# powdr-labs/powdr

Measured on AMD Instinct MI355X. Metric: STARK cells/sec (trace rows x cols) proving guest-keccak [bus interactions (LogUp) inside the proof], higher is better.
Workload: dtype u32 (BabyBear, Montgomery)

## Files before the change

include/powdr_prover.h:

```cpp
#ifndef POWDR_PROVER_H
#define POWDR_PROVER_H

#include <stddef.h>
#include <stdint.h>

#ifdef __cplusplus
extern "C" {
#endif

typedef struct PwProver PwProver;

typedef struct {
    uint32_t num_queries;
    uint32_t pow_bits;
} PwStarkConfig;

PwProver* pw_prover_create(const PwStarkConfig* cfg, uint32_t width, const uint32_t* cons_bytecode,
                           size_t bytecode_len, const uint32_t* cons_spans, size_t n_constraints);
PwProver* pw_prover_create_logup(const PwStarkConfig* cfg, uint32_t width, const uint32_t* cons_bytecode,
                                 size_t bytecode_len, const uint32_t* cons_spans, size_t n_constraints,
                                 const uint32_t* interactions, size_t n_interactions, const uint32_t* inter_spans,
                                 size_t n_inter_spans, const uint32_t* inter_bytecode, size_t inter_bytecode_len);
int pw_prover_trace_root(PwProver* p, const uint32_t* d_trace, uint32_t log_height, uint32_t* root8);
int pw_prover_set_bus_seed(PwProver* p, const uint32_t* seed8);
// ... 112 lines not shown

void pw_set_device_budget(size_t bytes);
size_t pw_get_device_budget(void);

int pw_prove_airs(const PwSegmentAir* airs, size_t n_airs, int shared_bus_seed, unsigned n_workers,
                  const uint32_t** proofs, size_t* n_words, uint32_t* bus_seed8);

typedef struct PwAirDescription {
    uint32_t width, log_height;
    uint32_t logup;
    const uint32_t* cons_bytecode; size_t bytecode_len;
    const uint32_t* cons_spans; size_t n_constraints;
    const uint32_t* interactions; size_t n_interactions;
    const uint32_t* inter_spans; size_t n_inter_spans;
    const uint32_t* inter_bytecode; size_t inter_bytecode_len;
} PwAirDescription;

int pw_verify_segment(const PwStarkConfig* cfg, const PwAirDescription* airs, size_t n_airs, int logup,
                      const uint32_t* proof_words, size_t n_words, int check_balance, uint32_t* total_sum4);

typedef struct PwAirPreprocessed {
    uint32_t width;
    uint32_t root8[8];
} PwAirPreprocessed;

int pw_verify_segment_preprocessed(const PwStarkConfig* cfg, const PwAirDescription* airs, const PwAirPreprocessed* pre, size_t n_airs,
                                   int logup, const uint32_t* proof_words, size_t n_words, int check_balance, uint32_t* total_sum4);

int pw_verify_segment_transition(const PwStarkConfig* cfg, const PwAirDescription* airs, const PwAirPreprocessed* pre, size_t n_airs,
                                 int logup, const uint32_t* proof_words, size_t n_words, int check_balance, uint32_t* total_sum4);

typedef struct PwAirPublic {
    uint32_t n;
    const uint32_t* expected;
} PwAirPublic;

int pw_verify_segment_public(const PwStarkConfig* cfg, const PwAirDescription* airs, const PwAirPreprocessed* pre, const PwAirPublic* pub,
                             size_t n_airs, int logup, const uint32_t* proof_words, size_t n_words, int check_balance, uint32_t* total_sum4);
size_t pw_segment_proof_public_values(const PwAirDescription* airs, const PwAirPublic* pub, size_t n_airs, const uint32_t* proof_words,
                                      size_t n_words, size_t air, uint32_t* out, size_t cap);

typedef struct PwChainSegment {
    const PwAirDescription* airs;
    const PwAirPreprocessed* pre;
    const PwAirPublic* pub;
    size_t n_airs;
    int logup;
    const uint32_t* proof;
    size_t n_words;
    int check_balance;
} PwChainSegment;
typedef struct PwChainLink {
    uint32_t air_from, index_from, air_to, index_to;
} PwChainLink;
int pw_verify_segment_chain(const PwStarkConfig* cfg, const PwChainSegment* segments, size_t n_segments, const PwChainLink* links,
                            size_t n_links, size_t* where);

int pw_verify_airs(const PwStarkConfig* cfg, const PwAirDescription* airs, size_t n_airs,
                   const uint32_t* const* proofs, const size_t* n_words, int shared_bus_seed, int check_balance,
                   uint32_t* total_sum4);

typedef int (*PwSegmentProveFn)(void* user, size_t segment, size_t worker, int device, uint32_t* commitment8);
int pw_prove_segments_multi(const int* devices, size_t n_workers, const uint64_t* segment_cells, size_t n_segments,
                            PwSegmentProveFn prove, void* user, uint32_t* commitments, uint32_t* worker_of_segment);
int pw_multi_last_merge(void);
size_t pw_assign_units(const uint64_t* cells, size_t n_units, size_t n_workers, uint32_t* worker_of_unit);

void pw_commitment_digest(const uint32_t* roots8, size_t n, uint32_t* digest8);

int pw_prover_reserve(PwProver* p, uint32_t log_height);

int pw_prover_stream_log_blocks(const PwProver* p, uint32_t log_height);

int pw_prover_max_constraint_degree(const PwProver* p);

int pw_prover_specialise(PwProver* p);
size_t pw_provers_specialise(PwProver* const* provers, size_t n);
int pw_prover_specialised(const PwProver* p, size_t* n_kernels, size_t* code_bytes, size_t* n_chunks);
size_t pw_jit_generated_source(uint32_t width, const uint32_t* cons_bytecode, size_t bytecode_len, const uint32_t* cons_spans, size_t n_constraints,
                               const uint32_t* interactions, size_t n_interactions, const uint32_t* inter_spans, size_t n_inter_spans,
                               const uint32_t* inter_bytecode, size_t inter_bytecode_len, int which, uint32_t chunk_cost, uint32_t chunks_per_unit,
                               size_t unit, char* buf, size_t cap, char* kernel_name, size_t name_cap, uint32_t* first_chunk, uint32_t* n_chunks,
                               uint32_t* total_chunks);
void pw_jit_cache_stats(uint64_t* units_compiled, uint64_t* units_from_disk);
int pw_jit_compile_check(uint32_t width, const uint32_t* cons_bytecode, size_t bytecode_len, const uint32_t* cons_spans, size_t n_constraints,
                         const uint32_t* interactions, size_t n_interactions, const uint32_t* inter_spans, size_t n_inter_spans,
                         const uint32_t* inter_bytecode, size_t inter_bytecode_len, size_t* n_kernels, size_t* code_bytes, size_t* n_chunks,
                         char* err, size_t err_cap);

uint32_t pw_prover_width(const PwProver* p);

size_t pw_prover_device_bytes(const PwProver* p);


int pw_lde_batch(const uint32_t* d_trace, uint32_t width, uint32_t log_height, uint32_t* d_coeffs, uint32_t* d_lde);

int pw_lde_fused(const uint32_t* d_trace, uint32_t width, uint32_t log_height, uint32_t* d_tmp, uint32_t* d_lde);

int pw_lde_subcoset(const uint32_t* d_coeffs, uint32_t width, uint32_t log_height, uint32_t log_blocks, uint32_t r, uint32_t* d_scale,
                    uint32_t* d_out);

int pw_merkle_commit(const uint32_t* d_matrix, size_t height, uint32_t width, uint32_t* d_digests);

void pw_poseidon2_permute_host(uint32_t* state16);

int pw_set_poseidon2_constants(const uint32_t* ext_rc, const uint32_t* int_rc);
void pw_get_poseidon2_constants(uint32_t* ext_rc, uint32_t* int_rc, uint32_t* diag);

#ifdef __cplusplus
}
#endif
#endif
```

powdr_amd/csrc/host/jit.cpp:

```cpp
#include "../jit.hpp"
#include "../common.hpp"

#include <dlfcn.h>
#include <fcntl.h>
#include <sys/file.h>
#include <spawn.h>
#include <sys/stat.h>
#include <sys/wait.h>
#include <unistd.h>

#include <atomic>
#include <cerrno>
#include <cstdio>
#include <cstdlib>
#include <cstring>
#include <iterator>
#include <map>
#include <mutex>
#include <thread>
#include <unordered_map>

extern char** environ;

namespace pw { namespace jit {
// ... 260 lines not shown
    if (!f) return;
    const uint64_t env = environment_hash(), src_len = source.size(), code_len = code.size();
    bool ok = fwrite(kDiskMagic, 1, 8, f) == 8 && fwrite(&env, 8, 1, f) == 1 && fwrite(&src_len, 8, 1, f) == 1 &&
              fwrite(source.data(), 1, source.size(), f) == source.size() && fwrite(&code_len, 8, 1, f) == 1 &&
              fwrite(code.data(), 1, code.size(), f) == code.size();
    ok = fclose(f) == 0 && ok;
    if (!ok || rename(tmp.c_str(), path.c_str()) != 0) (void)unlink(tmp.c_str());
}
}

bool compile_to_code_object(const std::string& source, std::vector<char>& code, std::string* err) { return compile_code(source, code, err); }

void cache_stats(uint64_t* compiled, uint64_t* from_disk) {
    if (compiled) *compiled = g_units_compiled.load();
    if (from_disk) *from_disk = g_units_from_disk.load();
}

bool available() {
    if (const char* e = getenv("POWDR_JIT")) if (atoi(e) == 0) return false;
    return rtc().ok;
}

std::vector<ProgramPtr> compile_all(const std::vector<std::string>& sources, std::string* err) {
    std::vector<ProgramPtr> out(sources.size());
    if (!rtc().ok) { if (err) *err = "hiprtc is not available"; return {}; }
    std::vector<size_t> todo;
    {
        std::lock_guard<std::mutex> lk(g_cache_mu);
        for (size_t i = 0; i < sources.size(); ++i) {
            auto it = g_cache.find(hash64(sources[i]));
            ProgramPtr hit = it != g_cache.end() ? it->second.lock() : nullptr;
            if (hit && hit->source == sources[i]) out[i] = hit;
            else todo.push_back(i);
        }
    }
    const std::string cache_dir = todo.empty() ? std::string() : disk_cache_dir();
    std::vector<std::pair<size_t, std::vector<char>>> from_disk;
    if (!cache_dir.empty()) {
        std::vector<size_t> still;
        for (size_t i : todo) {
            std::vector<char> c;
            if (disk_load(cache_dir, sources[i], c)) from_disk.emplace_back(i, std::move(c));
            else still.push_back(i);
        }
        todo.swap(still);
        g_units_from_disk += from_disk.size();
    }
    auto publish = [&](size_t i, std::vector<char>&& code_i) {
        auto p = std::make_shared<Program>();
        p->source = sources[i];
        p->code = std::move(code_i);
        std::weak_ptr<Program>& slot = g_cache[hash64(sources[i])];
        ProgramPtr other = slot.lock();
        if (other && other->source == sources[i]) out[i] = other;
        else { slot = p; out[i] = p; }
    };
    if (!from_disk.empty()) {
        std::lock_guard<std::mutex> lk(g_cache_mu);
        for (auto& e : from_disk) publish(e.first, std::move(e.second));
    }
    if (!todo.empty()) {
        DirLock lock(cache_dir);
        if (lock.fd >= 0) {
            std::vector<size_t> still;
            std::vector<std::pair<size_t, std::vector<char>>> late;
            for (size_t i : todo) {
                std::vector<char> c;
                if (disk_load(cache_dir, sources[i], c)) late.emplace_back(i, std::move(c));
                else still.push_back(i);
            }
            todo.swap(still);
            g_units_from_disk += late.size();
            std::lock_guard<std::mutex> lk(g_cache_mu);
            for (auto& e : late) publish(e.first, std::move(e.second));
        }
        if (!todo.empty()) {
            unsigned n_procs = std::thread::hardware_concurrency();
            if (n_procs > 32) n_procs = 32;
            if (const char* e = getenv("POWDR_JIT_THREADS")) { const int v = atoi(e); if (v >= 1 && v <= 256) n_procs = (unsigned)v; }
            if (n_procs < 1) n_procs = 1;
            if (n_procs > todo.size()) n_procs = (unsigned)todo.size();
            std::vector<std::vector<char>> code(todo.size());
            bool compiled = false;
            const std::string helper = n_procs > 1 ? helper_path() : std::string();
            std::string e;
            if (!helper.empty() && compile_with_helpers(helper, sources, todo, n_procs, code, compiled, &e)) {
                if (!compiled) { if (err) *err = e; return {}; }
            } else {
                for (size_t k = 0; k < todo.size(); ++k)
                    if (!compile_code(sources[todo[k]], code[k], &e)) { if (err) *err = e; return {}; }
            }
            g_units_compiled += todo.size();
            for (size_t k = 0; k < todo.size(); ++k) disk_store(cache_dir, sources[todo[k]], code[k]);
            std::lock_guard<std::mutex> lk(g_cache_mu);
            for (size_t k = 0; k < todo.size(); ++k) publish(todo[k], std::move(code[k]));
            if (g_cache.size() > 4096)
                for (auto it = g_cache.begin(); it != g_cache.end();) it = it->second.expired() ? g_cache.erase(it) : std::next(it);
        }
    }
    return out;
}

hipFunction_t kernel(Program& p, const char* name, std::string* err) {
    int device = 0;
    if (hipGetDevice(&device) != hipSuccess) { if (err) *err = "hipGetDevice failed"; return nullptr; }
    std::lock_guard<std::mutex> lk(p.mu);
    auto it = p.modules.find(device);
    if (it == p.modules.end()) {
        hipModule_t m = nullptr;
        const hipError_t e = hipModuleLoadData(&m, p.code.data());
        if (e != hipSuccess) { if (err) *err = std::string("hipModuleLoadData: ") + hipGetErrorString(e); (void)hipGetLastError(); return nullptr; }
        it = p.modules.emplace(device, m).first;
    }
    hipFunction_t f = nullptr;
    const hipError_t e = hipModuleGetFunction(&f, it->second, name);
    if (e != hipSuccess) { if (err) *err = std::string("hipModuleGetFunction(") + name + "): " + hipGetErrorString(e); (void)hipGetLastError(); return nullptr; }
    return f;
}

int launch(hipFunction_t f, dim3 grid, dim3 block, void** args, hipStream_t st) {
    return (int)hipModuleLaunchKernel(f, grid.x, grid.y, grid.z, block.x, block.y, block.z, 0, st, args, nullptr);
}

size_t code_bytes(const Program& p) { return p.code.size(); }

}}
```

powdr_amd/csrc/host/jit_codegen.cpp:

```cpp
#include "../jit_codegen.hpp"
#include "../xbc.hpp"

#include <cstdio>
#include <unordered_map>

namespace pw { namespace jit {

namespace {

struct Emitter {
    std::string& out;
    const char* matrix;
    std::unordered_map<uint32_t, uint32_t> loaded;
    uint32_t n_tmp = 0;
    explicit Emitter(std::string& o, const char* m) : out(o), matrix(m) {}

    std::string col(uint32_t c) {
        char b[96];
        if (!loaded.count(c)) {
            loaded[c] = 1;
            snprintf(b, sizeof b, "const uint32_t c%u = pwj::ld(%s + (size_t)%uu * N, j4);\n", c, matrix, c);
            out += b;
        }
        snprintf(b, sizeof b, "c%u", c);
        return b;
    }
    std::unordered_map<uint32_t, uint32_t> pub_loaded;
    std::string pubv(uint32_t k) {
        char b[96];
        if (!pub_loaded.count(k)) {
            pub_loaded[k] = 1;
            snprintf(b, sizeof b, "const uint32_t p%u = pub[%uu];\n", k, k);
            out += b;
        }
        snprintf(b, sizeof b, "p%u", k);
        return b;
    }
    static std::string lit(uint32_t m) { char b[24]; snprintf(b, sizeof b, "%uu", m); return b; }
    std::string tmp(const std::string& expr) {
        char b[32];
        snprintf(b, sizeof b, "t%u", n_tmp++);
        out += "const uint32_t ";
        out += b;
        out += " = " + expr + ";\n";
        return b;
    }
    bool expr(const uint32_t* code, uint32_t n_instr, std::string& value) {
        std::vector<std::string> stk;
        std::string top = "0u";
        auto bin = [&](const char* f, const std::string& a, const std::string& b) { return tmp(std::string("bb::") + f + "(" + a + ", " + b + ")"); };
        for (uint32_t ip = 0; ip < n_instr; ++ip) {
            const uint32_t op = code[2 * ip], a = code[2 * ip + 1];
            switch (op) {
                case xbc::SET_COL: top = col(a); break;
                case xbc::SET_CONST: top = lit(a); break;
                case xbc::PUSH_COL: stk.push_back(top); top = col(a); break;
                case xbc::PUSH_CONST: stk.push_back(top); top = lit(a); break;
                case xbc::ADD_COL: top = bin("add", top, col(a)); break;
                case xbc::SUB_COL: top = bin("sub", top, col(a)); break;
                case xbc::RSUB_COL: top = bin("sub", col(a), top); break;
                case xbc::MUL_COL: top = bin("mul", top, col(a)); break;
                case xbc::ADD_CONST: top = bin("add", top, lit(a)); break;
                case xbc::RSUB_CONST: top = bin("sub", lit(a), top); break;
                case xbc::MUL_CONST: top = bin("mul", top, lit(a)); break;
                case xbc::ADD: case xbc::SUB: case xbc::RSUB: case xbc::MUL: {
                    if (stk.empty()) return false;
                    const std::string s = stk.back();
                    stk.pop_back();
                    top = op == xbc::ADD ? bin("add", s, top) : op == xbc::SUB ? bin("sub", s, top) : op == xbc::RSUB ? bin("sub", top, s) : bin("mul", s, top);
                    break;
                }
                case xbc::SET_PUB: top = pubv(a); break;
                case xbc::PUSH_PUB: stk.push_back(top); top = pubv(a); break;
                case xbc::ADD_PUB: top = bin("add", top, pubv(a)); break;
                case xbc::SUB_PUB: top = bin("sub", top, pubv(a)); break;
                case xbc::RSUB_PUB: top = bin("sub", pubv(a), top); break;
                case xbc::MUL_PUB: top = bin("mul", top, pubv(a)); break;
                case xbc::NEG: top = tmp("bb::neg(" + top + ")"); break;
                case xbc::INV: top = tmp("bb::inv_or_zero(" + top + ")"); break;
                default: return false;
            }
        }
        if (!stk.empty()) return false;
        value = top;
        return true;
    }
};

const char* kPrologue =
    "// generated by libpowdr_gpu (csrc/host/jit_codegen.cpp)\n"
    "#include \"jit_device.hpp\"\n"
    "using bb::Ext;\n";

struct Chunk { uint32_t c0, c1, g0, g1; };

uint32_t group_cost(const LogupView& lg, uint32_t g) {
    uint32_t cost = 150;
    for (uint32_t i = lg.gstarts[g]; i < lg.gstarts[g + 1]; ++i) {
        const LogupInteraction& it = lg.inter[i];
        cost += 60 + 14 * it.n_args;
        for (uint32_t k = 0; k <= it.n_args; ++k) cost += 6 * lg.exprs.spans[2 * (it.first_span + k) + 1];
    }
    return cost;
}

bool emit_member(Emitter& e, const LogupView& lg, uint32_t i, uint32_t g, uint32_t k, std::string& m) {
    const LogupInteraction& it = lg.inter[i];
    const uint32_t* sp = lg.exprs.spans + 2 * (size_t)it.first_span;
    if (!e.expr(lg.exprs.code + 2 * (size_t)sp[0], sp[1], m)) return false;
    std::vector<std::string> args(it.n_args);
    for (uint32_t j = 0; j < it.n_args; ++j)
        if (!e.expr(lg.exprs.code + 2 * (size_t)sp[2 + 2 * j], sp[3 + 2 * j], args[j])) return false;
    char b[160];
    if (it.n_args) {
        snprintf(b, sizeof b, "const uint32_t a%u_%u[%u] = {", g, k, it.n_args);
        e.out += b;
        for (uint32_t j = 0; j < it.n_args; ++j) e.out += (j ? ", " : "") + args[j];
        snprintf(b, sizeof b, "};\nconst Ext d%u_%u = pwj::denominator<%u>(sd, %uu, blpow, a%u_%u);\n", g, k, it.n_args, it.bus_monty, g, k);
        e.out += b;
    } else {
        snprintf(b, sizeof b, "const Ext d%u_%u = pwj::denominator0(sd, %uu);\n", g, k, it.bus_monty);
        e.out += b;
    }
    return true;
}

std::vector<Chunk> cut(const XbcView* cons, const LogupView* lg, uint32_t chunk_cost, size_t& total_cost) {
    std::vector<Chunk> chunks;
    total_cost = 0;
    if (cons) {
        uint32_t c0 = 0, acc = 0;
        for (uint32_t c = 0; c < cons->n; ++c) {
            const uint32_t cost = 14 + 6 * cons->spans[2 * c + 1];
            if (acc && acc + cost > chunk_cost) { chunks.push_back({c0, c, 0, 0}); c0 = c; acc = 0; }
            acc += cost;
            total_cost += cost;
        }
        if (cons->n > c0) chunks.push_back({c0, cons->n, 0, 0});
    }
    if (lg) {
        uint32_t g0 = 0, acc = 0;
        for (uint32_t g = 0; g < lg->n_groups; ++g) {
            const uint32_t cost = group_cost(*lg, g);
            if (acc && acc + cost > chunk_cost) { chunks.push_back({0, 0, g0, g}); g0 = g; acc = 0; }
            acc += cost;
            total_cost += cost;
        }
        if (lg->n_groups > g0) chunks.push_back({0, 0, g0, lg->n_groups});
    }
    return chunks;
}

template <class Body>
Generated assemble(const std::vector<Chunk>& chunks, uint32_t chunks_per_unit, const char* kernel_prefix, const char* signature,
                   const char* kernel_head, const char* kernel_tail, Body&& body) {
    Generated out;
    out.n_chunks = (uint32_t)chunks.size();
    if (chunks_per_unit < 1) chunks_per_unit = 1;
    for (uint32_t u0 = 0; u0 < chunks.size(); u0 += chunks_per_unit) {
        const uint32_t u1 = std::min<uint32_t>(u0 + chunks_per_unit, (uint32_t)chunks.size());
        Unit unit;
        unit.first_chunk = u0;
        unit.n_chunks = u1 - u0;
        for (uint32_t k = u0; k < u1; ++k) {
            if (chunks[k].g1 <= chunks[k].g0) continue;
            if (unit.g1 <= unit.g0) { unit.g0 = chunks[k].g0; unit.g1 = chunks[k].g1; }
            else { unit.g0 = std::min(unit.g0, chunks[k].g0); unit.g1 = std::max(unit.g1, chunks[k].g1); }
        }
        unit.kernel = std::string(kernel_prefix) + std::to_string(u0);
        std::string& s = unit.source;
        s = kPrologue;
        s += "extern \"C\" __global__ __launch_bounds__(256) void " + unit.kernel + signature + " {\n" + kernel_head;
        s += "switch (blockIdx.y) {\n";
        for (uint32_t k = u0; k < u1; ++k) {
            s += "case " + std::to_string(k - u0) + ": {\n";
            if (!body(chunks[k], k, s)) return Generated{};
            s += "} break;\n";
        }
        s += "default: break;\n}\n";
        s += kernel_tail;
        s += "}\n";
        out.units.push_back(std::move(unit));
    }
    return out;
}

}

Generated gen_quotient(const XbcView& cons, const LogupView* lg, uint32_t chunk_cost, uint32_t chunks_per_unit) {
    size_t total = 0;
    const std::vector<Chunk> chunks = cut(&cons, lg, chunk_cost, total);
    const uint32_t nc = cons.n;
    bool has_pub = false;
    for (uint32_t c = 0; c < cons.n && !has_pub; ++c)
        for (uint32_t i = cons.spans[2 * c], end = i + cons.spans[2 * c + 1]; i < end && !has_pub; ++i) has_pub = cons.code[2 * (size_t)i] >= xbc::SET_PUB;
    auto body = [&](const Chunk& ch, uint32_t id, std::string& s) -> bool {
        Emitter e(s, "T");
        char b[256];
        if (ch.c1 > ch.c0) {
            s += "bb::ExtWideAcc acc;\n";
            for (uint32_t c = ch.c0; c < ch.c1; ++c) {
                std::string v;
                if (!e.expr(cons.code + 2 * (size_t)cons.spans[2 * c], cons.spans[2 * c + 1], v)) return false;
                snprintf(b, sizeof b, "acc.fma(apow[%u], %s);\n", c, v.c_str());
                s += b;
            }
            s += "const Ext r = acc.result();\n";
        } else {
            s += "const pwj::DenominatorSeeds sd = pwj::denominator_seeds(al);\nbb::ExtProductAcc wide;\n";
            for (uint32_t g = ch.g0; g < ch.g1; ++g) {
                const uint32_t i0 = lg->gstarts[g], i1 = lg->gstarts[g + 1], n = i1 - i0;
                snprintf(b, sizeof b, "const Ext q%u = {{pwj::ld(Pm + (size_t)%uu * N, j4), pwj::ld(Pm + (size_t)%uu * N, j4), pwj::ld(Pm + (size_t)%uu * N, j4), "
                                      "pwj::ld(Pm + (size_t)%uu * N, j4)}};\n", g, 4 * g, 4 * g + 1, 4 * g + 2, 4 * g + 3);
                s += b;
                std::vector<std::string> m(n);
                for (uint32_t k = 0; k < n; ++k) if (!emit_member(e, *lg, i0 + k, g, k, m[k])) return false;
                const std::string G = std::to_string(g);
                if (n == 0) {
                    s += "const Ext term" + G + " = q" + G + ";\n";
                } else if (n == 1) {
                    s += "Ext term" + G + " = bb::ext_mul(q" + G + ", d" + G + "_0);\nterm" + G + ".c[0] = bb::sub(term" + G + ".c[0], " + m[0] + ");\n";
                } else {
                    s += "Ext den" + G + " = bb::ext_mul(d" + G + "_0, d" + G + "_1);\n";
                    s += "Ext num" + G + " = pwj::scale2(d" + G + "_1, " + m[0] + ", d" + G + "_0, " + m[1] + ");\n";
                    for (uint32_t k = 2; k < n; ++k) {
                        const std::string D = "d" + G + "_" + std::to_string(k);
                        s += "num" + G + " = bb::ext_add(bb::ext_mul(num" + G + ", " + D + "), bb::ext_scale(den" + G + ", " + m[k] + "));\n";
                        s += "den" + G + " = bb::ext_mul(den" + G + ", " + D + ");\n";
                    }
                    s += "const Ext term" + G + " = bb::ext_sub(bb::ext_mul(q" + G + ", den" + G + "), num" + G + ");\n";
                }
                snprintf(b, sizeof b, "wide.fma(apow[%u], term%u);\n", nc + g, g);
                s += b;
            }
            s += "const Ext r = wide.result();\n";
        }
        snprintf(b, sizeof b, "uint32_t* o = part + (size_t)%uu * 4 * N;\npwj::st(o, j4, r.c[0]); pwj::st(o + N, j4, r.c[1]); pwj::st(o + 2 * N, j4, r.c[2]); "
                              "pwj::st(o + 3 * N, j4, r.c[3]);\n", id);
        s += b;
        return true;
    };
    Generated g = assemble(chunks, chunks_per_unit, "pwj_quotient_",
                           has_pub ? "(const uint32_t* __restrict__ T, const uint32_t* __restrict__ Pm, size_t N, const Ext* __restrict__ apow, Ext al, "
                                     "const Ext* __restrict__ blpow, uint32_t* __restrict__ part, const uint32_t* __restrict__ pub)"
                                   : "(const uint32_t* __restrict__ T, const uint32_t* __restrict__ Pm, size_t N, const Ext* __restrict__ apow, Ext al, "
                                     "const Ext* __restrict__ blpow, uint32_t* __restrict__ part)",
                           "const uint32_t j = blockIdx.x * 256u + threadIdx.x;\nif (j >= N) return;\nconst uint32_t j4 = j * 4u;\n", "", body);
    g.est_instructions = total;
    g.has_pub = has_pub;
    return g;
}

Generated gen_logup_perm(const LogupView& lg, uint32_t chunk_cost, uint32_t chunks_per_unit) {
    size_t total = 0;
    const std::vector<Chunk> chunks = cut(nullptr, &lg, chunk_cost, total);
    constexpr uint32_t kBatch = 4;
    auto body = [&](const Chunk& ch, uint32_t id, std::string& s) -> bool {
        Emitter e(s, "T");
        char b[320];
        s += "const pwj::DenominatorSeeds sd = pwj::denominator_seeds(al);\nExt sum = bb::ext_zero();\n";
        for (uint32_t gb = ch.g0; gb < ch.g1; gb += kBatch) {
            const uint32_t ge = std::min(ch.g1, gb + kBatch), nb = ge - gb;
            std::vector<std::vector<std::string>> m(nb);
            std::string any;
            for (uint32_t g = gb; g < ge; ++g) {
                const uint32_t i0 = lg.gstarts[g], n = lg.gstarts[g + 1] - i0;
                m[g - gb].resize(n);
                for (uint32_t k = 0; k < n; ++k) {
                    const uint32_t* sp = lg.exprs.spans + 2 * (size_t)lg.inter[i0 + k].first_span;
                    if (!e.expr(lg.exprs.code + 2 * (size_t)sp[0], sp[1], m[g - gb][k])) return false;
                    any += (any.empty() ? "" : " | ") + m[g - gb][k];
                }
                s += "Ext q" + std::to_string(g) + " = bb::ext_zero();\n";
            }
            s += "if ((" + (any.empty() ? std::string("0u") : any) + ") != 0u) {\n";
            {
                Emitter ei(s, "T");
                ei.loaded = e.loaded;
                ei.n_tmp = e.n_tmp;
                for (uint32_t g = gb; g < ge; ++g) {
                    const uint32_t i0 = lg.gstarts[g], n = lg.gstarts[g + 1] - i0;
                    const std::string G = std::to_string(g);
                    const std::vector<std::string>& mg = m[g - gb];
                    for (uint32_t k = 0; k < n; ++k) {
                        const LogupInteraction& it = lg.inter[i0 + k];
                        const uint32_t* sp = lg.exprs.spans + 2 * (size_t)it.first_span;
                        std::vector<std::string> args(it.n_args);
                        for (uint32_t j = 0; j < it.n_args; ++j)
                            if (!ei.expr(lg.exprs.code + 2 * (size_t)sp[2 + 2 * j], sp[3 + 2 * j], args[j])) return false;
                        if (it.n_args) {
                            snprintf(b, sizeof b, "const uint32_t a%u_%u[%u] = {", g, k, it.n_args);
                            s += b;
                            for (uint32_t j = 0; j < it.n_args; ++j) s += (j ? ", " : "") + args[j];
                            snprintf(b, sizeof b, "};\nconst Ext d%u_%u = pwj::denominator<%u>(sd, %uu, blpow, a%u_%u);\n", g, k, it.n_args, it.bus_monty, g, k);
                            s += b;
                        } else {
                            snprintf(b, sizeof b, "const Ext d%u_%u = pwj::denominator0(sd, %uu);\n", g, k, it.bus_monty);
                            s += b;
                        }
                    }
                    if (n == 0) {
                        s += "const Ext den" + G + " = bb::ext_one();\n";
                    } else if (n == 1) {
                        s += "const Ext den" + G + " = d" + G + "_0;\n";
                    } else {
                        s += "Ext den" + G + " = bb::ext_mul(d" + G + "_0, d" + G + "_1);\n";
                        s += "Ext num" + G + " = pwj::scale2(d" + G + "_1, " + mg[0] + ", d" + G + "_0, " + mg[1] + ");\n";
                        for (uint32_t k = 2; k < n; ++k) {
                            const std::string D = "d" + G + "_" + std::to_string(k);
                            s += "num" + G + " = bb::ext_add(bb::ext_mul(num" + G + ", " + D + "), bb::ext_scale(den" + G + ", " + mg[k] + "));\n";
                            s += "den" + G + " = bb::ext_mul(den" + G + ", " + D + ");\n";
                        }
                    }
                    s += "const pwj::ExtInvPrep ip" + G + " = pwj::ext_inv_prepare(den" + G + ");\n";
                }
                snprintf(b, sizeof b, "const uint32_t norms[%u] = {", nb);
                s += b;
                for (uint32_t g = gb; g < ge; ++g) s += std::string(g > gb ? ", " : "") + "ip" + std::to_string(g) + ".n";
                snprintf(b, sizeof b, "};\nuint32_t ninv[%u];\npwj::batch_inverse<%u>(norms, ninv);\n", nb, nb);
                s += b;
                for (uint32_t g = gb; g < ge; ++g) {
                    const uint32_t n = lg.gstarts[g + 1] - lg.gstarts[g];
                    const std::string G = std::to_string(g), inv = "pwj::ext_inv_finish(den" + G + ", ip" + G + ", ninv[" + std::to_string(g - gb) + "])";
                    if (n == 0) continue;
                    if (n == 1) s += "q" + G + " = bb::ext_scale(" + inv + ", " + m[g - gb][0] + ");\n";
                    else s += "q" + G + " = bb::ext_mul(num" + G + ", " + inv + ");\n";
                }
                e.n_tmp = ei.n_tmp;
            }
            s += "}\n";
            for (uint32_t g = gb; g < ge; ++g) {
                snprintf(b, sizeof b, "{ uint32_t* o = perm + (size_t)%uu * N; pwj::st(o, j4, q%u.c[0]); pwj::st(o + N, j4, q%u.c[1]); pwj::st(o + 2 * N, j4, q%u.c[2]); "
                                      "pwj::st(o + 3 * N, j4, q%u.c[3]); }\nsum = bb::ext_add(sum, q%u);\n", 4 * g, g, g, g, g, g);
                s += b;
            }
        }
        snprintf(b, sizeof b, "uint32_t* o = rowsum_part + (size_t)%uu * 4 * N;\npwj::st(o, j4, sum.c[0]); pwj::st(o + N, j4, sum.c[1]); pwj::st(o + 2 * N, j4, sum.c[2]); "
                              "pwj::st(o + 3 * N, j4, sum.c[3]);\n", id);
// ... 13 lines not shown
```

powdr_amd/csrc/jit_codegen.hpp:

```cpp
#pragma once
#include "prover_internal.hpp"

#include <string>
#include <vector>

namespace pw { namespace jit {

struct XbcView {
    const uint32_t* code;
    const uint32_t* spans;
    uint32_t n;
};
struct LogupView {
    const LogupInteraction* inter;
    uint32_t n_inter;
    XbcView exprs;
    const uint32_t* gstarts;
    uint32_t n_groups;
};

struct Unit {
    std::string source;
    std::string kernel;
    uint32_t first_chunk;
    uint32_t n_chunks;
    uint32_t g0 = 0, g1 = 0;
};
struct Generated {
    std::vector<Unit> units;
    uint32_t n_chunks = 0;
    size_t est_instructions = 0;
    bool has_pub = false;
};

Generated gen_quotient(const XbcView& cons, const LogupView* lg, uint32_t chunk_cost, uint32_t chunks_per_unit);

Generated gen_logup_perm(const LogupView& lg, uint32_t chunk_cost, uint32_t chunks_per_unit);

}}
```

powdr_amd/csrc/jit_device.hpp:

```cpp
#pragma once
#include "ext.hpp"

namespace pwj {

using bb::Ext;

__device__ __forceinline__ uint32_t ld(const uint32_t* __restrict__ base, uint32_t off4) {
    return *reinterpret_cast<const uint32_t*>(reinterpret_cast<const char*>(base) + off4);
}
__device__ __forceinline__ void st(uint32_t* __restrict__ base, uint32_t off4, uint32_t v) {
    *reinterpret_cast<uint32_t*>(reinterpret_cast<char*>(base) + off4) = v;
}

struct DenominatorSeeds {
    int64_t s[4];
    uint32_t al0;
};
__device__ __forceinline__ DenominatorSeeds denominator_seeds(const Ext& al) {
    DenominatorSeeds sd;
#pragma unroll
    for (int k = 0; k < 4; ++k) sd.s[k] = (int64_t)bb::centred(al.c[k]) * (int64_t)bb::R_MOD_P;
    sd.al0 = al.c[0];
    return sd;
}
struct DenominatorAcc {
    int64_t T[4];
    uint32_t pending;
    __device__ __forceinline__ DenominatorAcc(const DenominatorSeeds& sd, uint32_t bus_monty)
        : T{(int64_t)bb::centred(bb::add(sd.al0, bus_monty)) * (int64_t)bb::R_MOD_P, sd.s[1], sd.s[2], sd.s[3]}, pending(0) {}
    __device__ __forceinline__ void reduce() {
#pragma unroll
        for (int k = 0; k < 4; ++k) T[k] = bb::smul_uniform(bb::smont(T[k]), (int32_t)bb::R_MOD_P);
        pending = 0;
    }
    __device__ __forceinline__ void add(uint32_t a, const Ext& b) {
        if (pending == 2) reduce();
#pragma unroll
        for (int k = 0; k < 4; ++k) T[k] = bb::swide_mad_uniform(T[k], (int32_t)a, bb::centred(b.c[k]));
        ++pending;
    }
    __device__ __forceinline__ Ext result() {
        if (pending == 2) reduce();
        Ext d;
#pragma unroll
        for (int k = 0; k < 4; ++k) {
            const uint32_t x = (uint32_t)bb::smont(T[k]);
            d.c[k] = bb::umin(x, x + bb::P);
        }
        return d;
    }
};
template <int NA>
__device__ __forceinline__ Ext denominator(const DenominatorSeeds& sd, uint32_t bus_monty, const Ext* __restrict__ blpow, const uint32_t (&a)[NA]) {
    DenominatorAcc acc(sd, bus_monty);
#pragma unroll
    for (int j = 0; j < NA; ++j) acc.add(a[j], blpow[j + 1]);
    return acc.result();
}
__device__ __forceinline__ Ext denominator0(const DenominatorSeeds& sd, uint32_t bus_monty) {
    DenominatorAcc acc(sd, bus_monty);
    return acc.result();
}

__device__ __forceinline__ Ext scale2(const Ext& a, uint32_t x, const Ext& b, uint32_t y) {
    return {{bb::mul2(a.c[0], x, b.c[0], y), bb::mul2(a.c[1], x, b.c[1], y), bb::mul2(a.c[2], x, b.c[2], y), bb::mul2(a.c[3], x, b.c[3], y)}};
}

struct ExtInvPrep { uint32_t d0, d1, n; };
__device__ __forceinline__ ExtInvPrep ext_inv_prepare(const Ext& a) {
    const uint32_t W = bb::w11();
    const uint32_t s0 = bb::add(bb::sqr(a.c[0]), bb::mul(W, bb::sqr(a.c[2])));
    const uint32_t s1 = bb::double_(bb::mul(a.c[0], a.c[2]));
    const uint32_t t0 = bb::add(bb::sqr(a.c[1]), bb::mul(W, bb::sqr(a.c[3])));
    const uint32_t t1 = bb::double_(bb::mul(a.c[1], a.c[3]));
    ExtInvPrep p;
    p.d0 = bb::sub(s0, bb::mul(W, t1));
    p.d1 = bb::sub(s1, t0);
    p.n = bb::sub(bb::sqr(p.d0), bb::mul(W, bb::sqr(p.d1)));
    return p;
}
__device__ __forceinline__ Ext ext_inv_finish(const Ext& a, const ExtInvPrep& p, uint32_t n_inv) {
    const uint32_t W = bb::w11();
    const uint32_t e0 = bb::mul(p.d0, n_inv);
    const uint32_t e1 = bb::neg(bb::mul(p.d1, n_inv));
    const uint32_t r00 = bb::add(bb::mul(a.c[0], e0), bb::mul(W, bb::mul(a.c[2], e1)));
    const uint32_t r01 = bb::add(bb::mul(a.c[0], e1), bb::mul(a.c[2], e0));
    const uint32_t r10 = bb::neg(bb::add(bb::mul(a.c[1], e0), bb::mul(W, bb::mul(a.c[3], e1))));
    const uint32_t r11 = bb::neg(bb::add(bb::mul(a.c[1], e1), bb::mul(a.c[3], e0)));
    return {{r00, r10, r01, r11}};
}
template <int K>
__device__ __forceinline__ void batch_inverse(const uint32_t (&n)[K], uint32_t (&out)[K]) {
    uint32_t x[K], pre[K];
#pragma unroll
    for (int i = 0; i < K; ++i) {
        x[i] = n[i] == 0u ? bb::R_MOD_P : n[i];
        pre[i] = i ? bb::mul(pre[i - 1], x[i]) : x[i];
    }
    uint32_t inv = bb::inv(pre[K - 1]);
#pragma unroll
    for (int i = K - 1; i > 0; --i) {
        out[i] = bb::mul(inv, pre[i - 1]);
        inv = bb::mul(inv, x[i]);
    }
    out[0] = inv;
}

}
```

powdr_amd/csrc/logup_kernels.hip:

```cpp
#include "prover_internal.hpp"
#include "xbc.hpp"
#include "expr_eval.hpp"
#include "jit_device.hpp"
#include "logup_eval.hpp"

namespace pw {

namespace {

constexpr int kBlock = kLogupBlock;
using bb::Ext;


using pwj::DenominatorSeeds;
using pwj::denominator_seeds;
template <bool FAST>
__device__ __forceinline__ Ext interaction_denominator(const LogupInteraction& it, const LogupProgram& lp, const uint32_t* __restrict__ m,
                                                       size_t stride, size_t r, uint32_t* stk, const DenominatorSeeds& sd,
                                                       const Ext* __restrict__ blpow) {
    pwj::DenominatorAcc acc(sd, it.bus_monty);
    for (uint32_t j = 0; j < it.n_args; ++j) acc.add(eval_span<FAST>(lp, it.first_span + 1 + j, m, stride, r, stk), blpow[j + 1]);
    return acc.result();
}
template <bool FAST>
// ... 11 lines not shown
    const size_t r = (size_t)blockIdx.x * kBlock + threadIdx.x;
    if (r >= H) return;
    const DenominatorSeeds sd = denominator_seeds(al);
    Ext acc = bb::ext_zero();
    for (uint32_t g = 0; g < lp.n_groups; ++g) {
        Ext num = bb::ext_zero(), den = bb::ext_one();
        bool any = false;
        for (uint32_t i = lp.d_gstarts[g]; i < lp.d_gstarts[g + 1]; ++i) {
            const LogupInteraction it = lp.d_inter[i];
            const uint32_t m = interaction_mult<FAST>(it, lp, trace, H, r, stk);
            if (m == 0u) continue;
            const Ext d = interaction_denominator<FAST>(it, lp, trace, H, r, stk, sd, blpow);
            if (any) {
                num = bb::ext_add(bb::ext_mul(num, d), bb::ext_scale(den, m));
                den = bb::ext_mul(den, d);
            } else {
                num = bb::ext_from_base(m);
                den = d;
                any = true;
            }
        }
        const Ext q = any ? bb::ext_mul(num, bb::ext_inv(den)) : bb::ext_zero();
        uint32_t* out = perm + (size_t)(4 * g) * H + r;
        out[0] = q.c[0]; out[H] = q.c[1]; out[2 * H] = q.c[2]; out[3 * H] = q.c[3];
        acc = bb::ext_add(acc, q);
    }
    rowsum[r] = acc;
}

constexpr int kScanPerThread = 16;
constexpr int kScanChunk = kBlock * kScanPerThread;

__device__ __forceinline__ Ext block_exclusive_scan(Ext v, Ext* lds, Ext& total) {
    const int t = threadIdx.x;
    lds[t] = v;
    __syncthreads();
    for (int off = 1; off < kBlock; off <<= 1) {
        Ext x = lds[t];
        if (t >= off) x = bb::ext_add(x, lds[t - off]);
        __syncthreads();
        lds[t] = x;
        __syncthreads();
    }
    total = lds[kBlock - 1];
    Ext incl = lds[t];
    __syncthreads();
    return bb::ext_sub(incl, v);
}

__global__ __launch_bounds__(kBlock) void scan_block_totals_kernel(const Ext* __restrict__ in, size_t H, Ext* __restrict__ totals) {
    __shared__ Ext lds[kBlock];
    const size_t base = (size_t)blockIdx.x * kScanChunk + (size_t)threadIdx.x * kScanPerThread;
    Ext s = bb::ext_zero();
    for (int k = 0; k < kScanPerThread; ++k)
        if (base + k < H) s = bb::ext_add(s, in[base + k]);
    Ext total;
    (void)block_exclusive_scan(s, lds, total);
    if (threadIdx.x == 0) totals[blockIdx.x] = total;
}
__global__ void scan_totals_kernel(Ext* totals, uint32_t n) {
    if (threadIdx.x == 0 && blockIdx.x == 0) {
        Ext run = bb::ext_zero();
        for (uint32_t i = 0; i < n; ++i) { Ext t = totals[i]; totals[i] = run; run = bb::ext_add(run, t); }
    }
}
__global__ __launch_bounds__(kBlock) void scan_write_kernel(const Ext* __restrict__ in, size_t H, const Ext* __restrict__ offsets,
                                                             uint32_t* __restrict__ phi_cols ) {
    __shared__ Ext lds[kBlock];
    const size_t base = (size_t)blockIdx.x * kScanChunk + (size_t)threadIdx.x * kScanPerThread;
    Ext s = bb::ext_zero();
    for (int k = 0; k < kScanPerThread; ++k)
        if (base + k < H) s = bb::ext_add(s, in[base + k]);
    Ext total;
    Ext run = bb::ext_add(block_exclusive_scan(s, lds, total), offsets[blockIdx.x]);
    for (int k = 0; k < kScanPerThread; ++k) {
        if (base + k < H) {
            run = bb::ext_add(run, in[base + k]);
            phi_cols[base + k] = run.c[0]; phi_cols[H + base + k] = run.c[1];
            phi_cols[2 * H + base + k] = run.c[2]; phi_cols[3 * H + base + k] = run.c[3];
        }
    }
}

template <bool XBC, bool FAST, bool PUB>
__global__ __launch_bounds__(kBlock) void quotient_logup_kernel(const uint32_t* __restrict__ lde, const uint32_t* __restrict__ plde,
                                                                 size_t N, const uint32_t* __restrict__ bytecode,
                                                                 const uint32_t* __restrict__ spans, uint32_t nc, LogupProgram lp,
                                                                 const Ext* __restrict__ apow, Ext al, const Ext* __restrict__ blpow,
                                                                 Ext S, uint32_t zval_even, uint32_t zval_odd, uint32_t shift,
                                                                 uint32_t wN, uint32_t ginv, uint32_t* __restrict__ q, int main_only,
                                                                 const uint32_t* __restrict__ pub, uint32_t pub_base) {
    __shared__ uint32_t stack_lds[kStackCap * kBlock];
    uint32_t* stk = stack_lds + threadIdx.x;
    const size_t j = (size_t)blockIdx.x * kBlock + threadIdx.x;
    if (j >= N) return;
    const size_t jn = (j + 2) & (N - 1);
    const DenominatorSeeds sd = denominator_seeds(al);
    bb::ExtProductAcc wide;
    for (uint32_t c = 0; c < nc; ++c) {
        const uint32_t off = spans[2 * c], len = spans[2 * c + 1];
        const uint32_t v = XBC ? xbc::eval<kBlock, true, PUB>(bytecode + 2 * (size_t)off, len, lde, j, stk, N, pub)
                               : eval_expr<kBlock, true, PUB>(bytecode + off, len, lde, j, stk, N, pub, pub_base);
        wide.fma_base(apow[c], v);
    }
    Ext sumq = bb::ext_zero(), sumq_next = bb::ext_zero();
    for (uint32_t g = 0; g < lp.n_groups; ++g) {
        const uint32_t* pc = plde + (size_t)(4 * g) * N;
        const Ext qi = {{pc[j], pc[N + j], pc[2 * N + j], pc[3 * N + j]}};
        if (!main_only) {
            const Ext qn = {{pc[jn], pc[N + jn], pc[2 * N + jn], pc[3 * N + jn]}};
            sumq = bb::ext_add(sumq, qi);
            sumq_next = bb::ext_add(sumq_next, qn);
        }
        const uint32_t i0 = lp.d_gstarts[g], i1 = lp.d_gstarts[g + 1];
        Ext num, den;
        for (uint32_t i = i0; i < i1; ++i) {
            const LogupInteraction it = lp.d_inter[i];
            const Ext d = interaction_denominator<FAST>(it, lp, lde, N, j, stk, sd, blpow);
            const uint32_t m = interaction_mult<FAST>(it, lp, lde, N, j, stk);
            if (i == i0) {
                num = bb::ext_from_base(m);
                den = d;
            } else {
                num = bb::ext_add(bb::ext_mul(num, d), bb::ext_scale(den, m));
                den = bb::ext_mul(den, d);
            }
        }
        wide.fma(apow[nc + g], bb::ext_sub(bb::ext_mul(qi, den), num));
    }
    Ext acc = wide.result();
    if (main_only) {
#pragma unroll
        for (int k = 0; k < 4; ++k) q[(size_t)k * N + j] = acc.c[k];
        return;
    }
    const uint32_t* pp = plde + (size_t)(4 * lp.n_groups) * N;
    const Ext phi = {{pp[j], pp[N + j], pp[2 * N + j], pp[3 * N + j]}};
    const Ext phin = {{pp[jn], pp[N + jn], pp[2 * N + jn], pp[3 * N + jn]}};
    const uint32_t x = bb::mul(shift, bb::pow_u32(wN, (uint32_t)j));
    const uint32_t Z = (j & 1) ? zval_odd : zval_even;
    const uint32_t one = bb::R_MOD_P;
    const uint32_t is_first = bb::mul(Z, bb::inv(bb::sub(x, one)));
    const uint32_t is_last = bb::mul(Z, bb::inv(bb::sub(x, ginv)));
    const uint32_t is_trans = bb::sub(x, ginv);
    acc = bb::ext_add(acc, bb::ext_mul(apow[nc + lp.n_groups], bb::ext_scale(bb::ext_sub(phi, sumq), is_first)));
    acc = bb::ext_add(acc, bb::ext_mul(apow[nc + lp.n_groups + 1], bb::ext_scale(bb::ext_sub(bb::ext_sub(phin, phi), sumq_next), is_trans)));
    acc = bb::ext_add(acc, bb::ext_mul(apow[nc + lp.n_groups + 2], bb::ext_scale(bb::ext_sub(phi, S), is_last)));
    const uint32_t zi = bb::inv(Z);
#pragma unroll
    for (int k = 0; k < 4; ++k) q[(size_t)k * N + j] = bb::mul(acc.c[k], zi);
}

__global__ __launch_bounds__(kBlock) void quotient_logup_tail_kernel(const uint32_t* __restrict__ part, uint32_t n_chunks,
                                                                      const uint32_t* __restrict__ plde_phi, const uint32_t* __restrict__ plde_sumq,
                                                                      size_t N, const Ext* __restrict__ apow_tail, Ext S, uint32_t zval_even,
                                                                      uint32_t zval_odd, uint32_t shift, uint32_t wN, uint32_t ginv,
                                                                      uint32_t* __restrict__ q) {
    const size_t j = (size_t)blockIdx.x * kBlock + threadIdx.x;
    if (j >= N) return;
    const size_t jn = (j + 2) & (N - 1);
    Ext acc;
#pragma unroll
    for (int k = 0; k < 4; ++k) {
        uint64_t a = 0;
        for (uint32_t c = 0; c < n_chunks; ++c) a += part[((size_t)c * 4 + k) * N + j];
        acc.c[k] = (uint32_t)(a % bb::P);
// ... 81 lines not shown
        a1 = bb::ext_add(a1, row);
        a2 = bb::ext_add(a2, bb::ext_mul(gK, row));
    }
    const uint32_t xj = bb::mul(shift, bb::pow_u32(wN, (uint32_t)j));
    const Ext xe = bb::ext_from_base(xj);
    const Ext t1 = bb::ext_mul(bb::ext_sub(a1, sum1), bb::ext_inv(bb::ext_sub(xe, zeta)));
    const Ext t2 = bb::ext_mul(bb::ext_sub(a2, sum2), bb::ext_inv(bb::ext_sub(xe, gzeta)));
    v[j] = bb::ext_add(t1, t2);
}

}

int logup_scan(const bb::Ext* d_rowsum, size_t H, bb::Ext* d_block_totals, uint32_t* phi_cols) {
    const uint32_t blocks = div_up(H, kScanChunk);
    ScopedKernelTimer t("logup_scan_kernels");
    hipLaunchKernelGGL(scan_block_totals_kernel, dim3(blocks), dim3(kBlock), 0, stream(), d_rowsum, H, d_block_totals);
    hipLaunchKernelGGL(scan_totals_kernel, dim3(1), dim3(64), 0, stream(), d_block_totals, blocks);
    hipLaunchKernelGGL(scan_write_kernel, dim3(blocks), dim3(kBlock), 0, stream(), d_rowsum, H, d_block_totals, phi_cols);
    return (int)hipGetLastError();
}

int logup_perm_trace(const uint32_t* trace, size_t H, const LogupProgram& lp, bb::Ext al, const bb::Ext* d_blpow, uint32_t* perm,
                     bb::Ext* d_rowsum, bb::Ext* d_block_totals) {
    {
        ScopedKernelTimer t("logup_perm_kernel");
        call_stats()[kStatInterpreterKernelLaunches] += 1;
        if (lp.d_forms) hipLaunchKernelGGL(logup_perm_kernel<true>, dim3(div_up(H, kBlock)), dim3(kBlock), 0, stream(), trace, H, lp, al, d_blpow, perm, d_rowsum);
        else hipLaunchKernelGGL(logup_perm_kernel<false>, dim3(div_up(H, kBlock)), dim3(kBlock), 0, stream(), trace, H, lp, al, d_blpow, perm, d_rowsum);
    }
    return logup_scan(d_rowsum, H, d_block_totals, perm + (size_t)(4 * lp.n_groups) * H);
}

int logup_rowsum_combine(const uint32_t* part, uint32_t n_chunks, size_t H, bb::Ext* d_rowsum, uint32_t* cols4) {
    ScopedKernelTimer t("logup_rowsum_combine_kernel");
    hipLaunchKernelGGL(rowsum_combine_kernel, dim3(div_up(H, kBlock)), dim3(kBlock), 0, stream(), part, n_chunks, H, d_rowsum, cols4);
    return (int)hipGetLastError();
}

int quotient_logup_tail(const uint32_t* part, uint32_t n_chunks, const uint32_t* plde_phi, const uint32_t* plde_sumq, size_t N, int logN,
                        const bb::Ext* d_apow_tail, bb::Ext S, uint32_t zval_even, uint32_t zval_odd, uint32_t* q) {
    const uint32_t shift = bb::to_monty(field::kCosetShift), wN = field::root_of_unity(logN);
    const uint32_t ginv = bb::inv(field::root_of_unity(logN - 1));
    ScopedKernelTimer t("quotient_logup_tail_kernel");
    hipLaunchKernelGGL(quotient_logup_tail_kernel, dim3(div_up(N, kBlock)), dim3(kBlock), 0, stream(), part, n_chunks, plde_phi, plde_sumq, N,
                       d_apow_tail, S, zval_even, zval_odd, shift, wN, ginv, q);
    return (int)hipGetLastError();
}

int quotient_eval_logup(const uint32_t* lde, const uint32_t* plde, size_t N, int logN, const ConstraintProgram& prog,
                        const LogupProgram& lp, const bb::Ext* d_apow, bb::Ext al, const bb::Ext* d_blpow, bb::Ext S,
                        uint32_t zval_even, uint32_t zval_odd, uint32_t* q, bool main_only) {
    const uint32_t shift = bb::to_monty(field::kCosetShift), wN = field::root_of_unity(logN);
    const uint32_t ginv = bb::inv(field::root_of_unity(logN - 1));
    const int mo = main_only ? 1 : 0;
    ScopedKernelTimer t("quotient_logup_kernel");
    call_stats()[kStatInterpreterKernelLaunches] += 1;
#define PW_LAUNCH_QL2(X, F, P) hipLaunchKernelGGL((quotient_logup_kernel<X, F, P>), dim3(div_up(N, kBlock)), dim3(kBlock), 0, stream(), lde, plde, N, \
                                                prog.d_bytecode, prog.d_spans, prog.n_constraints, lp, d_apow, al, d_blpow, S, zval_even, zval_odd, shift, wN, \
                                                ginv, q, mo, prog.d_pub, prog.pub_base)
#define PW_LAUNCH_QL(X, F) do { if (prog.d_pub) PW_LAUNCH_QL2(X, F, true); else PW_LAUNCH_QL2(X, F, false); } while (0)
    if (prog.is_xbc) { if (lp.d_forms) PW_LAUNCH_QL(true, true); else PW_LAUNCH_QL(true, false); }
    else { if (lp.d_forms) PW_LAUNCH_QL(false, true); else PW_LAUNCH_QL(false, false); }
#undef PW_LAUNCH_QL2
#undef PW_LAUNCH_QL
    return (int)hipGetLastError();
}

int deep_quotient_logup(const uint32_t* lde, uint32_t W, const uint32_t* plde, uint32_t Wp, const uint32_t* qlde, size_t N, int logN,
                        const bb::Ext* d_gpow, bb::Ext sum1, bb::Ext sum2, bb::Ext zeta, bb::Ext gzeta, bb::Ext* v) {
    ScopedKernelTimer t("deep_logup_kernel");
    hipLaunchKernelGGL(deep_logup_kernel<false>, dim3(div_up(N, kBlock)), dim3(kBlock), 0, stream(), lde, W, plde, Wp, qlde, N, d_gpow, sum1,
                       sum2, zeta, gzeta, bb::to_monty(field::kCosetShift), field::root_of_unity(logN), bb::ext_zero(), v);
    return (int)hipGetLastError();
}

int deep_quotient_two_point(const uint32_t* lde, uint32_t W, const uint32_t* plde, uint32_t Wp, const uint32_t* qlde, size_t N, int logN,
                            const bb::Ext* d_gpow, bb::Ext gK, bb::Ext sum1, bb::Ext sum2, bb::Ext zeta, bb::Ext gzeta, bb::Ext* v) {
    ScopedKernelTimer t("deep_two_point_kernel");
    hipLaunchKernelGGL(deep_logup_kernel<true>, dim3(div_up(N, kBlock)), dim3(kBlock), 0, stream(), lde, W, plde, Wp, qlde, N, d_gpow, sum1,
                       sum2, zeta, gzeta, bb::to_monty(field::kCosetShift), field::root_of_unity(logN), gK, v);
    return (int)hipGetLastError();
}

}
```

powdr_amd/csrc/prover.hip:

```cpp
#include "prover_state.hpp"
#include "prover_stages.hpp"
#include "xbc_compile.hpp"

#include <atomic>
#include <cstdlib>
#include <cstring>
#include <algorithm>
#include <initializer_list>
#include <vector>

namespace pw {

namespace {

__global__ void gather_records_kernel(const uint32_t* __restrict__ arena, const uint64_t* __restrict__ offsets,
                                      uint32_t words_per_record, uint32_t n, uint32_t* __restrict__ out) {
    const uint32_t i = blockIdx.x * blockDim.x + threadIdx.x;
    if (i >= n * words_per_record) return;
    const uint32_t r = i / words_per_record, w = i - r * words_per_record;
    out[i] = arena[offsets[r] + w];
}

}

int gather_records(const uint32_t* arena, const uint64_t* d_offsets, uint32_t words_per_record, uint32_t n, uint32_t* out) {
    if (!n) return 0;
    hipLaunchKernelGGL(gather_records_kernel, dim3(div_up((size_t)n * words_per_record, 256)), dim3(256), 0, stream(), arena, d_offsets,
                       words_per_record, n, out);
    return (int)hipGetLastError();
}

}

using namespace pw;

extern "C" void pw_prover_destroy(PwProver* p);
extern "C" size_t pw_prover_device_bytes(const PwProver* p);
extern "C" int pw_prover_specialise(PwProver* p);
extern "C" int pw_prover_specialised(const PwProver* p, size_t* n_kernels, size_t* code_bytes, size_t* n_chunks);

static std::vector<uint32_t> remap_row_programs(const uint32_t* bc, const uint32_t* spans, size_t n_constraints, uint32_t w1, uint32_t flags,
                                                std::vector<uint32_t>& next_cols, uint32_t* row_cols, std::vector<uint32_t>& new_spans) {
    next_cols.clear();
    for (size_t k = 0; k < n_constraints; ++k)
        for (uint32_t ip = spans[2 * k], end = spans[2 * k] + spans[2 * k + 1]; ip < end;) {
            const uint32_t op = bc[ip++];
            if (op != POWDR_OP_PUSH_APC && op != POWDR_OP_PUSH_CONST) continue;
            const uint32_t a = bc[ip++];
            if (op == POWDR_OP_PUSH_APC && a >= w1 && a < 2 * w1) next_cols.push_back(a - w1);
        }
    std::sort(next_cols.begin(), next_cols.end());
    next_cols.erase(std::unique(next_cols.begin(), next_cols.end()), next_cols.end());
    auto slot = [&](uint32_t c) { return (uint32_t)(std::lower_bound(next_cols.begin(), next_cols.end(), c) - next_cols.begin()); };
    const uint32_t n_next = (uint32_t)next_cols.size();
    *row_cols = n_next + ((flags & pw::kRowsSelector) ? 3u : 0u);
    std::vector<uint32_t> out;
    new_spans.clear();
    for (size_t k = 0; k < n_constraints; ++k) {
        new_spans.push_back((uint32_t)out.size());
        new_spans.push_back(spans[2 * k + 1]);
        for (uint32_t ip = spans[2 * k], end = spans[2 * k] + spans[2 * k + 1]; ip < end;) {
            const uint32_t op = bc[ip++];
            out.push_back(op);
            if (op != POWDR_OP_PUSH_APC && op != POWDR_OP_PUSH_CONST) continue;
            uint32_t a = bc[ip++];
            if (op == POWDR_OP_PUSH_APC && a >= 2 * w1 + 3) a = w1 + *row_cols + (a - (2 * w1 + 3));
            else if (op == POWDR_OP_PUSH_APC && a >= w1) a = a < 2 * w1 ? w1 + slot(a - w1) : w1 + n_next + (a - 2 * w1);
            out.push_back(a);
        }
    }
    return out;
}

static PwProver* create_prover(const PwStarkConfig* cfg, uint32_t width, const uint32_t* bc, size_t bc_len,
                               const uint32_t* spans, size_t n_constraints, bool device, uint32_t rows_w1 = 0, uint32_t n_public = 0) {
    if (!cfg || !width || (n_public && !rows_w1)) return nullptr;
    PwProver* p = new PwProver();
    p->cfg = *cfg;
    p->width = width;
    p->n_constraints = (uint32_t)n_constraints;
    p->h_spans.assign(spans, spans + 2 * n_constraints);
    const uint32_t bound = rows_w1 ? 2 * rows_w1 + 3 + n_public : width, deg0 = rows_w1 ? 2 * rows_w1 + 2 : 0xffffffffu;
    const uint32_t deg0_from = n_public ? 2 * rows_w1 + 3 : 0xffffffffu;
    p->n_public = n_public;
    for (size_t k = 0; k < n_constraints; ++k) {
// ... 189 lines not shown
    return create_row_prover(cfg, width, pre_width, log_height, d_pre, n_public, bc, bc_len, spans, n_constraints, inter, n_inter, ispans, n_ispans,
                             ibc, ibc_len, true);
}

extern "C" uint32_t pw_prover_n_public(const PwProver* p) { return p ? p->n_public : 0; }

extern "C" int pw_prover_set_public_values(PwProver* p, const uint32_t* values, size_t n) {
    if (!p || n != p->n_public || (n && !values)) return -1;
    for (size_t k = 0; k < n; ++k) if (values[k] >= bb::P) return -1;
    p->h_pub.resize(n);
    for (size_t k = 0; k < n; ++k) p->h_pub[k] = bb::to_monty(values[k]);
    p->pub_set = true;
    return 0;
}

extern "C" int pw_public_programs_check(uint32_t width, uint32_t pre_width, uint32_t n_public, const uint32_t* bc, size_t bc_len,
                                        const uint32_t* spans, size_t n_constraints, const uint32_t* inter, size_t n_inter,
                                        const uint32_t* ispans, size_t n_ispans, const uint32_t* ibc, size_t ibc_len, int* max_degree,
                                        uint32_t* row_flags, uint32_t* xbc_out, size_t xbc_cap, size_t* xbc_len, char* src, size_t src_cap,
                                        size_t* src_len) {
    const PwStarkConfig cfg{1, 0};
    PwProver* p = create_row_prover(&cfg, width, pre_width, 0, nullptr, n_public, bc, bc_len, spans, n_constraints, inter, n_inter, ispans, n_ispans,
                                    ibc, ibc_len, false);
    if (!p) return -2;
    if (max_degree) *max_degree = p->max_degree;
    if (row_flags) *row_flags = p->row_flags;
    if (xbc_len) *xbc_len = p->h_xcode.size();
    for (size_t i = 0; xbc_out && i < p->h_xcode.size() && i < xbc_cap; ++i) xbc_out[i] = p->h_xcode[i];
    std::string all;
    for (const pw::jit::Unit& u : pw::generate_sources(p, 0, 8000, 8).units) all += u.source;
    if (src_len) *src_len = all.size();
    if (src && src_cap) { strncpy(src, all.c_str(), src_cap - 1); src[src_cap - 1] = 0; }
    pw_prover_destroy(p);
    return 0;
}

extern "C" uint32_t pw_prover_row_flags(const PwProver* p) { return p ? p->row_flags : 0; }
namespace pw {
bool prover_segment_only(const PwProver* p) { return p && (p->pre_width || p->transition || p->n_public); }
}

extern "C" int pw_prover_preprocessed_root(const PwProver* p, uint32_t* root8) {
    if (!p || !root8 || !p->pre_width) return -1;
    for (int k = 0; k < 8; ++k) root8[k] = p->pre_root[k];
    return 0;
}

extern "C" uint32_t pw_prover_preprocessed_width(const PwProver* p) { return p ? p->pre_width : 0; }

extern "C" int pw_jit_compile_check(uint32_t width, const uint32_t* bc, size_t bc_len, const uint32_t* spans, size_t n_constraints,
                                    const uint32_t* inter, size_t n_inter, const uint32_t* ispans, size_t n_ispans, const uint32_t* ibc,
                                    size_t ibc_len, size_t* n_kernels, size_t* code_bytes, size_t* n_chunks, char* err, size_t err_cap) {
    const PwStarkConfig cfg{1, 0};
    PwProver* p = inter ? create_prover_logup(&cfg, width, bc, bc_len, spans, n_constraints, inter, n_inter, ispans, n_ispans, ibc, ibc_len, false)
                        : create_prover(&cfg, width, bc, bc_len, spans, n_constraints, false);
    if (!p) return -2;
    const int rc = pw_prover_specialise(p);
    (void)pw_prover_specialised(p, n_kernels, code_bytes, n_chunks);
    if (err && err_cap) { strncpy(err, p->jit.error.c_str(), err_cap - 1); err[err_cap - 1] = 0; }
    pw_prover_destroy(p);
    return rc;
}

extern "C" size_t pw_jit_generated_source(uint32_t width, const uint32_t* bc, size_t bc_len, const uint32_t* spans, size_t n_constraints,
                                          const uint32_t* inter, size_t n_inter, const uint32_t* ispans, size_t n_ispans, const uint32_t* ibc,
                                          size_t ibc_len, int which, uint32_t chunk_cost, uint32_t chunks_per_unit, size_t unit, char* buf, size_t cap,
                                          char* kernel_name, size_t name_cap, uint32_t* first_chunk, uint32_t* n_chunks, uint32_t* total_chunks) {
    const PwStarkConfig cfg{1, 0};
    PwProver* p = inter ? create_prover_logup(&cfg, width, bc, bc_len, spans, n_constraints, inter, n_inter, ispans, n_ispans, ibc, ibc_len, false)
                        : create_prover(&cfg, width, bc, bc_len, spans, n_constraints, false);
    if (!p) return 0;
    const pw::jit::Generated g = pw::generate_sources(p, which, chunk_cost ? chunk_cost : 8000, chunks_per_unit ? chunks_per_unit : 8);
    pw_prover_destroy(p);
    if (total_chunks) *total_chunks = g.n_chunks;
    if (unit >= g.units.size()) return 0;
    const pw::jit::Unit& u = g.units[unit];
    if (buf && cap) { strncpy(buf, u.source.c_str(), cap - 1); buf[cap - 1] = 0; }
    if (kernel_name && name_cap) { strncpy(kernel_name, u.kernel.c_str(), name_cap - 1); kernel_name[name_cap - 1] = 0; }
    if (first_chunk) *first_chunk = u.first_chunk;
    if (n_chunks) *n_chunks = u.n_chunks;
    return u.source.size();
}

#define TRY(x) do { int _rc = (x); if (_rc) return _rc; } while (0)

extern "C" int pw_prover_logup_path(const PwProver* p) { return !p || !p->logup ? 0 : p->d_iforms ? 2 : 1; }

extern "C" int pw_prover_set_bus_seed(PwProver* p, const uint32_t* seed8) {
    if (!p || !p->logup) return (int)hipErrorInvalidValue;
    p->has_bus_seed = seed8 != nullptr;
    if (seed8) for (int i = 0; i < 8; ++i) p->bus_seed[i] = bb::to_monty(seed8[i] % bb::P);
    return 0;
}

namespace pw {
size_t lde_panel_cols(size_t H, size_t widest) {
    int panel_log_words = 28;
    if (const char* e = getenv("POWDR_PANEL_LOG_WORDS")) { const int v = atoi(e); if (v >= 12 && v <= 32) panel_log_words = v; }
    size_t cols = ((size_t)1 << panel_log_words) / H;
    if (cols < 8) cols = 8;
    if (cols > widest) cols = widest;
    return cols ? cols : 1;
}
int lde_matrix(PwProver* p, const CommitLayout& L, uint32_t log_h, const uint32_t* m, uint32_t cols, uint32_t* out) {
    uint32_t* d_coef = p->coef.as<uint32_t>();
    for (size_t c0 = 0; c0 < cols; c0 += L.panel_cols) {
        const uint32_t pc = (uint32_t)(cols - c0 < L.panel_cols ? cols - c0 : L.panel_cols);
        const char* ef = getenv("POWDR_LDE_FUSED");
        const bool fused = ef ? atoi(ef) != 0 : (log_h <= 12 || (log_h >= 15 && log_h <= 20));
        if (!fused) {
            TRY(intt_dif(m + c0 * L.H, d_coef, L.H, L.H, pc, (int)log_h));
            TRY(coset_lde_from_coeffs(d_coef, out + c0 * L.N, L.H, L.N, pc, (int)log_h));
        } else {
            TRY(lde_fused(m + c0 * L.H, d_coef, out + c0 * L.N, L.H, L.H, L.N, pc, (int)log_h));
        }
    }
    return 0;
}
}

namespace {


void plan_buffers(const PwProver* p, uint32_t log_h, int b, CommitLayout& L, BufferPlan& B, bool consume = false) {
    const AirShape s = air_shape(p, log_h, p->logup);
    const bool lg = p->logup;
    plan_stage_buffers(p, s, AirMode{b, b && consume}, L, B);
    L.tree_words = merkle_words(s.N);
    L.fri_words = FriLayout(s.logN).fri_words;
    L.n_trees = lg ? 3 : 2;
    B.digests = (L.n_trees * L.tree_words + L.fri_words) * 4;
    if (b) { B.tcoef = consume ? 0 : (size_t)s.W * s.H * 4; B.fscale = (size_t)1 << 15; }
    B.ext_arena = (2 * s.N + (lg ? 3 : 1) * s.H + s.H / 4096 + 32) * sizeof(bb::Ext);
    const size_t misc_ext = dot_scratch_words(s) + 2 * (size_t)s.K + s.M + p->max_args + 64;
    const uint32_t nq = p->cfg.num_queries;
    const size_t path_records = (size_t)nq * (L.n_trees * (size_t)s.logN + (size_t)log_h * s.logN) + 16;
    B.misc = misc_ext * sizeof(bb::Ext) + (size_t)nq * 8 + (size_t)nq * s.K1 * 4 + path_records * (8 + 32) + (size_t)nq * log_h * (8 + 16) + 4096;
}

}

namespace pw {
static std::atomic<size_t> g_device_budget{(size_t)-1};
size_t device_budget() {
    size_t b = g_device_budget.load();
    if (b == (size_t)-1) {
        const char* e = getenv("POWDR_DEVICE_BUDGET_BYTES");
        b = e ? (size_t)strtoull(e, nullptr, 10) : 0;
        g_device_budget.store(b);
    }
    return b;
}
bool device_room(size_t held, size_t* avail) {
    size_t free_b = 0, total_b = 0;
    if (hipMemGetInfo(&free_b, &total_b) != hipSuccess) { (void)hipGetLastError(); return false; }
    const size_t others = total_b > free_b + held ? total_b - free_b - held : 0;
    size_t a = (size_t)((double)(free_b + held) * 0.92);
    const size_t cap = (size_t)((double)total_b * 0.90);
    a = std::min(a, cap > others ? cap - others : (size_t)0);
    if (const size_t budget = device_budget()) a = std::min(a, budget);
    *avail = a;
    return true;
}
}

extern "C" void pw_set_device_budget(size_t bytes) { pw::g_device_budget.store(bytes); }
// ... 46 lines not shown
        TRY(merkle_commit_matrix(p->lde.as<uint32_t>(), L.N, p->width, L.N, d_tdig));
    }
    PW_HIP_TRY(hipMemcpyAsync(root, d_tdig + L.tree_words - 8, 32, hipMemcpyDeviceToHost, st));
    PW_HIP_TRY(hipStreamSynchronize(st));
    return 0;
}


int ensure_prove_buffers(PwProver* p, uint32_t log_h, int b, CommitLayout& L, bool consume = false) {
    BufferPlan B;
    plan_buffers(p, log_h, b, L, B, consume);
    return apply_buffers(p, B);
}
}

namespace pw {
size_t proof_plan_bytes(const PwProver* p, uint32_t log_h, int b, bool consume) {
    CommitLayout L;
    BufferPlan B;
    plan_buffers(p, log_h, b, L, B, consume && b > 0);
    return B.total();
}
int ensure_proof_buffers(PwProver* p, uint32_t log_h, int b, CommitLayout& L, bool consume) {
    return ensure_prove_buffers(p, log_h, b, L, consume && b > 0);
}
}

extern "C" int pw_prover_trace_root(PwProver* p, const uint32_t* d_trace, uint32_t log_h, uint32_t* root8) {
    if (!p || !d_trace || !root8 || log_h < 1 || log_h > 26) return (int)hipErrorInvalidValue;
    if (p->pre_width || p->transition || p->n_public) return -1;
    (void)hipGetLastError();
    TRY(poseidon2_upload_params());
    CommitLayout L;
    p->committed_trace = nullptr;
    (void)specialise_provers(&p, 1, &log_h, false);
    const int sb = stream_log_blocks(p, log_h);
    if (sb < 0) return (int)hipErrorOutOfMemory;
    TRY(ensure_commit_buffers(p, log_h, sb, L));
    TRY(commit_trace(p, L, d_trace, log_h, p->committed_root));
    for (int i = 0; i < 8; ++i) root8[i] = bb::from_monty(p->committed_root[i]);
    p->committed_trace = d_trace;
    p->committed_log_h = log_h;
    p->committed_b = sb;
    return (int)hipGetLastError();
}

static void release_opened_mailbox(PwProver* p) {
    PwProver::OpenedMailbox& mb = p->opened_mb;
    for (int i = 0; i < mb.n_events; ++i) (void)hipEventDestroy(mb.ev[i]);
    mb.n_events = 0;
    if (mb.host) (void)hipHostFree(mb.host);
    mb.host = mb.dev = nullptr;
    mb.cap = 0;
    mb.device = -1;
}

static PwProver::OpenedMailbox* opened_mailbox(PwProver* p, size_t K) {
    const char* env = getenv("POWDR_OPENINGS_OVERLAP");
    if (env && atoi(env) == 0) return nullptr;
    PwProver::OpenedMailbox& mb = p->opened_mb;
    int device = 0;
    if (hipGetDevice(&device) != hipSuccess) { (void)hipGetLastError(); return nullptr; }
    if (mb.host && (mb.device != device || mb.cap < K)) release_opened_mailbox(p);
    if (!mb.host) {
        void *h = nullptr, *d = nullptr;
        const size_t cap = std::max<size_t>(K, 64);
        if (hipHostMalloc(&h, cap * sizeof(bb::Ext), hipHostMallocMapped) != hipSuccess) { (void)hipGetLastError(); return nullptr; }
        if (hipHostGetDevicePointer(&d, h, 0) != hipSuccess) { (void)hipGetLastError(); (void)hipHostFree(h); return nullptr; }
        mb.host = (bb::Ext*)h; mb.dev = (bb::Ext*)d; mb.cap = cap; mb.device = device;
        while (mb.n_events < PwProver::OpenedMailbox::kEvents) {
            if (hipEventCreateWithFlags(&mb.ev[mb.n_events], hipEventDisableTiming) != hipSuccess) {
                (void)hipGetLastError();
                release_opened_mailbox(p);
                return nullptr;
            }
            ++mb.n_events;
        }
    }
    return &mb;
}

extern "C" void pw_prover_destroy(PwProver* p) {
    if (!p) return;
    for (DeviceBuf* b : {&p->coef, &p->lde, &p->digests, &p->q, &p->qcoef, &p->qlde, &p->ext_arena, &p->misc, &p->perm, &p->plde, &p->qpart, &p->tcoef,
                         &p->fscale, &p->gbuf, &p->pre_vals, &p->pre_lde, &p->pre_tree, &p->row_vals, &p->bus_order})
        b->release();
    if (p->d_next_cols) (void)hipFree(p->d_next_cols);
    if (p->d_pub) (void)hipFree(p->d_pub);
    for (void* q : {(void*)p->d_inter, (void*)p->d_ixspans, (void*)p->d_icode, (void*)p->d_gstarts, (void*)p->d_iforms}) if (q) (void)hipFree(q);
    if (p->d_bytecode) (void)hipFree(p->d_bytecode);
    if (p->d_spans) (void)hipFree(p->d_spans);
    release_opened_mailbox(p);
    delete p;
}

extern "C" uint32_t pw_prover_width(const PwProver* p) { return p ? p->width : 0; }
extern "C" int pw_prover_max_constraint_degree(const PwProver* p) { return p ? p->max_degree : -1; }

extern "C" int pw_prover_reserve(PwProver* p, uint32_t log_h) {
    if (!p || log_h < 1 || log_h > 26) return (int)hipErrorInvalidValue;
    (void)hipGetLastError();
    CommitLayout L;
    (void)specialise_provers(&p, 1, &log_h, false);
    const int sb = stream_log_blocks(p, log_h);
    if (sb < 0) return (int)hipErrorOutOfMemory;
    return ensure_prove_buffers(p, log_h, sb, L);
}

extern "C" int pw_prover_stream_log_blocks(const PwProver* p, uint32_t log_h) {
    if (!p || log_h < 1 || log_h > 26) return -1;
    return stream_log_blocks(p, log_h);
}

extern "C" size_t pw_prover_device_bytes(const PwProver* p) {
    return p->coef.bytes + p->lde.bytes + p->digests.bytes + p->q.bytes + p->qcoef.bytes + p->qlde.bytes +
           p->ext_arena.bytes + p->misc.bytes + p->perm.bytes + p->plde.bytes + p->qpart.bytes + p->tcoef.bytes + p->fscale.bytes + p->gbuf.bytes +
           p->pre_vals.bytes + p->pre_lde.bytes + p->pre_tree.bytes + p->row_vals.bytes + p->bus_order.bytes;
}


namespace {
int prove_impl(PwProver* p, const uint32_t* d_trace, uint32_t log_h, const uint32_t** proof_words, size_t* n_words, bool consume) {
    if (!p || !d_trace || log_h < 1 || log_h > 26 || p->pre_width || p->transition || p->n_public) return -1;
    if (consume && ((uintptr_t)d_trace & 15)) return (int)hipErrorInvalidValue;
    (void)hipGetLastError();
    const AirShape s = air_shape(p, log_h, p->logup);
    const uint32_t W = s.W, nc = s.nc, n_int = s.n_int, Wp = s.Wp, K1 = s.K1, K = s.K, M = s.M;
    const size_t H = s.H, N = s.N;
    const int logN = s.logN;
    const bool lg = p->logup;
    hipStream_t st = stream();
    TRY(poseidon2_upload_params());
    (void)specialise_provers(&p, 1, &log_h, false);

    bool have_commitment = !consume && p->committed_trace == d_trace && p->committed_log_h == log_h;
    p->committed_trace = nullptr;
    int sb = have_commitment ? p->committed_b : stream_log_blocks(p, log_h, consume);
    if (sb < 0) return (int)hipErrorOutOfMemory;
    CommitLayout L;
    int rc_buf = ensure_prove_buffers(p, log_h, sb, L, consume && sb > 0);
    if (rc_buf == (int)hipErrorOutOfMemory && have_commitment && sb == 0) {
        (void)hipGetLastError();
        p->lde.release();
        have_commitment = false;
        sb = stream_log_blocks(p, log_h, false);
        if (sb <= 0) return (int)hipErrorOutOfMemory;
        rc_buf = ensure_prove_buffers(p, log_h, sb, L, false);
    }
    if (rc_buf) return rc_buf;
    const AirMode mode{sb, consume && sb > 0};
    const bool eat = mode.eat;
    const size_t tree_words = L.tree_words, n_trees = L.n_trees;
    uint32_t* d_tcoef = eat ? const_cast<uint32_t*>(d_trace) : p->tcoef.as<uint32_t>();
    const uint32_t nq = p->cfg.num_queries;

    uint32_t* d_lde = p->lde.as<uint32_t>();
    uint32_t* d_dig = p->digests.as<uint32_t>();
    uint32_t* d_qdig = d_dig + tree_words;
    uint32_t* d_pdig = d_dig + 2 * tree_words;
    uint32_t* d_fdig = d_dig + n_trees * tree_words;
    uint32_t* d_perm = p->perm.as<uint32_t>();
    uint32_t* d_plde = p->plde.as<uint32_t>();
    uint32_t* d_qlde = p->qlde.as<uint32_t>();
    bb::Ext* d_v = p->ext_arena.as<bb::Ext>();
    bb::Ext* d_weights = d_v + 2 * N;
    bb::Ext* d_scratch = p->misc.as<bb::Ext>();
    bb::Ext* d_opened = d_scratch + dot_scratch_words(s);
    bb::Ext* d_gpow = d_opened + K;
    bb::Ext* d_apow = d_gpow + K;
    bb::Ext* d_blpow = d_apow + M + 4;
    uint8_t* d_tail = reinterpret_cast<uint8_t*>(d_blpow + p->max_args + 8);
    const AirBufs bufs{d_trace, d_trace, d_tcoef, d_apow, d_blpow, d_weights, d_weights + H, d_weights + 2 * H, d_scratch};

    std::vector<uint32_t>& pf = p->proof;
    pf.clear();
    auto put = [&](uint32_t canonical) { pf.push_back(canonical); };
    auto put_monty = [&](const uint32_t* w, size_t n) { for (size_t i = 0; i < n; ++i) pf.push_back(bb::from_monty(w[i])); };

    Challenger ch;
    if (lg) {
        for (uint32_t x : {kMagic2 % bb::P, log_h, W, nc, n_int, p->cfg.num_queries, p->cfg.pow_bits}) ch.observe_canonical(x);
        for (uint32_t x : {kMagic2, log_h, W, nc, n_int, p->cfg.num_queries, p->cfg.pow_bits}) put(x);
    } else {
        for (uint32_t x : {kMagic % bb::P, log_h, W, nc, p->cfg.num_queries, p->cfg.pow_bits}) ch.observe_canonical(x);
        for (uint32_t x : {kMagic, log_h, W, nc, p->cfg.num_queries, p->cfg.pow_bits}) put(x);
    }

    uint32_t root[8];
    uint32_t* d_coef_tmp = eat ? (lg ? p->perm.as<uint32_t>() : d_tcoef) : nullptr;
    if (have_commitment) memcpy(root, p->committed_root, 32);
    else if (eat) {
        TRY(intt_dif(d_trace, d_coef_tmp, H, H, W, (int)log_h));
        TRY(commit_coefficients(p, L, log_h, d_coef_tmp, W, p->digests.as<uint32_t>()));
        PW_HIP_TRY(hipMemcpyAsync(root, p->digests.as<uint32_t>() + tree_words - 8, 32, hipMemcpyDeviceToHost, st));
        PW_HIP_TRY(hipStreamSynchronize(st));
    } else TRY(commit_trace(p, L, d_trace, log_h, root));
    put_monty(root, 8);
    ch.observe_words(root, 8);

// ... 305 lines not shown
```

powdr_amd/csrc/prover_internal.hpp:

```cpp
#pragma once
#include "babybear.hpp"
#include "ext.hpp"
#include "small_form.hpp"
#include "poseidon2.hpp"
#include "common.hpp"

#include <stddef.h>
#include <stdint.h>

struct PwProver;

namespace pw {

namespace field {
constexpr uint32_t kTwoAdicGen = 0x1a427a41u;
constexpr uint32_t kCosetShift = 31u;
inline uint32_t root_of_unity(int n) {
    uint32_t g = bb::to_monty(kTwoAdicGen);
    for (int i = n; i < 27; ++i) g = bb::sqr(g);
    return g;
}
}

int intt_dif(const uint32_t* in, uint32_t* out, size_t in_stride, size_t out_stride, uint32_t cols, int n);
// ... 11 lines not shown

const p2::Params& poseidon2_params_host();
int poseidon2_set_constants(const uint32_t* ext_rc128, const uint32_t* int_rc13);
int poseidon2_upload_params();
int merkle_commit_matrix(const uint32_t* m, size_t height, uint32_t width, size_t col_stride, uint32_t* digests, uint32_t* root_out = nullptr);
int merkle_leaf_hash(const uint32_t* m, size_t height, uint32_t width, size_t col_stride, uint32_t* digests, size_t digest_stride,
                     size_t digest_offset);
int merkle_build_levels(uint32_t* digests, size_t n_leaves, uint32_t* root_out = nullptr);
int merkle_leaf_absorb(const uint32_t* m, size_t col_stride, const uint32_t* const* d_cols, uint32_t n_cols, uint32_t pos0, size_t height, size_t rstride,
                       size_t roff, uint32_t* state, uint32_t* digests, bool first, bool last);
uint32_t* merkle_root_mailbox(uint32_t** device_ptr);
struct MixedLevelCols {
    const uint32_t* const* d_cols;
    uint32_t n_cols;
    uint32_t external = 0;
};
int merkle_commit_mixed(const MixedLevelCols* by_log, int L, uint32_t* digests, uint32_t* d_inject);
int merkle_commit_ext_pairs(const bb::Ext* v, size_t half, uint32_t* digests, uint32_t* root_out = nullptr);
inline size_t merkle_words(size_t n_leaves) { return (2 * n_leaves - 1) * 8; }
inline size_t merkle_level_offset(size_t n_leaves, int level) {
    size_t off = 0, n = n_leaves;
    for (int l = 0; l < level; ++l) { off += n * 8; n >>= 1; }
    return off;
}

bool prover_segment_only(const ::PwProver* p);

struct ConstraintProgram {
    const uint32_t* d_bytecode;
    const uint32_t* d_spans;
    uint32_t n_constraints;
    bool is_xbc;
    const uint32_t* d_pub = nullptr;
    uint32_t pub_base = 0xffffffffu;
};
uint32_t quotient_chunks(size_t N, uint32_t n_constraints);
int quotient_eval(const uint32_t* lde, size_t N, const ConstraintProgram& prog, const bb::Ext* d_alpha_pows,
                  uint32_t zinv_even, uint32_t zinv_odd, uint32_t* q, uint32_t* part, uint32_t n_chunks);
int quotient_combine(const uint32_t* part, uint32_t n_chunks, size_t N, uint32_t zinv_even, uint32_t zinv_odd, uint32_t* q);
int check_constraints(const uint32_t* trace, size_t H, const ConstraintProgram& prog, unsigned long long* d_first_and_count);
int row_layout_columns(uint32_t* m, size_t n, int log_n, uint32_t w1, const uint32_t* d_next_cols, uint32_t n_next, uint32_t step,
                       bool selectors, bool trace_domain);
int quotient_split(const uint32_t* cbr, size_t H, int log_h, uint32_t* out);
int zeta_weights(bb::Ext z, int log_h, bb::Ext* weights);
int barycentric_weights(bb::Ext zeta, int log_h, bb::Ext* weights);
int ext_dot_columns(const uint32_t* cols, size_t stride, uint32_t n_cols, size_t len, const bb::Ext* weights, bb::Ext* out,
                    bb::Ext* scratch);
int ext_dot_columns2(const uint32_t* cols, size_t stride, uint32_t n_cols, size_t len, const bb::Ext* weights, const bb::Ext* weights2,
                     bb::Ext* out, bb::Ext* out2, bb::Ext* scratch);
int deep_quotient(const uint32_t* lde_a, uint32_t wa, const uint32_t* lde_b, uint32_t wb, size_t N, int logN,
                  const bb::Ext* d_gpow, bb::Ext opened_sum, bb::Ext zeta, bb::Ext* v);
int ext_powers(bb::Ext base, uint32_t n, bool reversed, bool centred, bb::Ext* d_out);
int gamma_powers(bb::Ext gamma, uint32_t K, bb::Ext* d_gpow);
struct GatherRowsJob { const uint32_t* m; uint64_t height; uint32_t width; uint32_t idx_off; uint64_t out_off; };
int gather_rows_multi(const GatherRowsJob* d_jobs, uint32_t n_jobs, uint32_t max_width, const uint32_t* d_indices, uint32_t n_idx, uint32_t* out);
int fri_fold(const bb::Ext* v, size_t half, int log_size, uint32_t shift, bb::Ext beta, bb::Ext* out);
int ext_axpy(bb::Ext* y, const bb::Ext* a_or_null, const bb::Ext* x, size_t n);
int canonicalize_words(uint32_t* d_words, size_t n);
int gather_words(const uint32_t* const* d_ptrs, uint32_t n, uint32_t* d_out);
int gather_rows(const uint32_t* m, size_t height, uint32_t width, const uint32_t* d_indices, uint32_t n_idx, uint32_t* out);
struct LogupInteraction {
    uint32_t bus_monty;
    uint32_t n_args;
    uint32_t first_span;
};
struct LogupProgram {
    const LogupInteraction* d_inter;
    uint32_t n;
    const uint32_t* d_xspans;
    const uint32_t* d_code;
    const uint32_t* d_gstarts;
    uint32_t n_groups;
    const SmallForm* d_forms;
};
int logup_perm_trace(const uint32_t* trace, size_t H, const LogupProgram& lp, bb::Ext al, const bb::Ext* d_blpow, uint32_t* perm,
                     bb::Ext* d_rowsum, bb::Ext* d_block_totals);
int logup_scan(const bb::Ext* d_rowsum, size_t H, bb::Ext* d_block_totals, uint32_t* phi_cols);
int logup_rowsum_combine(const uint32_t* part, uint32_t n_chunks, size_t H, bb::Ext* d_rowsum, uint32_t* cols4);
int quotient_logup_tail(const uint32_t* part, uint32_t n_chunks, const uint32_t* plde_phi, const uint32_t* plde_sumq, size_t N, int logN,
                        const bb::Ext* d_apow_tail, bb::Ext S, uint32_t zval_even, uint32_t zval_odd, uint32_t* q);
int quotient_eval_logup(const uint32_t* lde, const uint32_t* plde, size_t N, int logN, const ConstraintProgram& prog,
                        const LogupProgram& lp, const bb::Ext* d_apow, bb::Ext al, const bb::Ext* d_blpow, bb::Ext S,
                        uint32_t zval_even, uint32_t zval_odd, uint32_t* q, bool main_only = false);
int deep_quotient_logup(const uint32_t* lde, uint32_t W, const uint32_t* plde, uint32_t Wp, const uint32_t* qlde, size_t N, int logN,
                        const bb::Ext* d_gpow, bb::Ext sum1, bb::Ext sum2, bb::Ext zeta, bb::Ext gzeta, bb::Ext* v);
int deep_quotient_two_point(const uint32_t* lde, uint32_t W, const uint32_t* plde, uint32_t Wp, const uint32_t* qlde, size_t N, int logN,
                            const bb::Ext* d_gpow, bb::Ext gK, bb::Ext sum1, bb::Ext sum2, bb::Ext zeta, bb::Ext gzeta, bb::Ext* v);

int part_scatter(const uint32_t* part, uint32_t n_chunks, size_t m, int b, uint32_t r, size_t N, uint32_t* out);
int ext_lincomb(const uint32_t* ma, uint32_t wa, const uint32_t* mb, uint32_t wb, size_t len, const bb::Ext* d_gpow, uint32_t second,
                uint32_t* out);
int deep_from_combo(const uint32_t* glde, const uint32_t* qlde, size_t N, int logN, const bb::Ext* d_gpow_quotient, bb::Ext sum1, bb::Ext sum2,
                    bb::Ext zeta, bb::Ext gzeta, int two, bb::Ext* v);
int ext_to_cols(const bb::Ext* in, size_t len, uint32_t* cols4);

int pow_grind(const uint32_t* state16, const uint32_t* pending, uint32_t in_len, uint32_t bits, uint32_t* d_best,
              uint32_t* witness_out);

}
```

powdr_amd/csrc/prover_jit.hip:

```cpp
#include "prover_state.hpp"

#include <algorithm>
#include <cstdlib>
#include <thread>

#define PW_TRY_INT(x) do { const int _rc = (x); if (_rc) return _rc; } while (0)

namespace pw {

namespace {

uint32_t env_u32(const char* name, uint32_t dflt, uint32_t lo, uint32_t hi) {
    if (const char* e = getenv(name)) { const long v = atol(e); if (v >= (long)lo && v <= (long)hi) return (uint32_t)v; }
    return dflt;
}

jit::LogupView logup_view(const PwProver* p) {
    return jit::LogupView{p->h_inter.data(), (uint32_t)p->h_inter.size(), jit::XbcView{p->h_icode.data(), p->h_ixspans.data(), (uint32_t)(p->h_ixspans.size() / 2)},
                          p->h_gstarts.data(), p->n_groups};
}

int launch_unit(const jit::Generated& g, const std::vector<jit::ProgramPtr>& progs, size_t u, size_t rows, void** args) {
    std::string err;
    hipFunction_t f = jit::kernel(*progs[u], g.units[u].kernel.c_str(), &err);
// ... 25 lines not shown
    return {};
}

int specialise_provers(PwProver* const* ps, size_t n, const uint32_t* log_heights, bool force) {
    const char* e = getenv("POWDR_JIT");
    const bool always = force || (e && atoi(e) == 1);
    const uint32_t min_log = env_u32("POWDR_JIT_MIN_LOG_HEIGHT", 18, 1, 40);
    const uint32_t chunk_cost = env_u32("POWDR_JIT_CHUNK_COST", 8000, 200, 1000000);
    const uint32_t per_unit_max = env_u32("POWDR_JIT_UNIT_CHUNKS", 8, 1, 4096);
    unsigned hw = std::thread::hardware_concurrency();
    hw = hw > 32 ? 32 : hw < 1 ? 1 : hw;
    auto per_unit_for = [&](size_t cost) {
        const size_t chunks = cost / chunk_cost + 1;
        const size_t want = (chunks + hw - 1) / hw;
        return (uint32_t)(want < 1 ? 1 : want > per_unit_max ? per_unit_max : want);
    };
    std::vector<PwProver*> todo;
    for (size_t i = 0; i < n; ++i) {
        PwProver* p = ps[i];
        if (!p || p->jit.state != 0) continue;
        if (!always && (!log_heights || log_heights[i] < min_log)) continue;
        if (!jit::available() || !p->is_xbc || (p->n_constraints == 0 && !p->logup)) { p->jit.state = -1; p->jit.error = "not available"; continue; }
        const jit::XbcView cons{p->h_xcode.data(), p->h_xspans.data(), p->n_constraints};
        const uint32_t per_unit = per_unit_for(6 * (p->h_xcode.size() / 2 + p->h_icode.size() / 2) + 300 * (size_t)p->n_groups);
        if (p->logup) {
            const jit::LogupView lv = logup_view(p);
            p->jit.quotient = jit::gen_quotient(cons, &lv, chunk_cost, per_unit);
            p->jit.perm = jit::gen_logup_perm(lv, chunk_cost, per_unit);
            if (p->n_groups && p->jit.perm.units.empty()) { p->jit.state = -1; p->jit.error = "code generation failed"; continue; }
        } else {
            p->jit.quotient = jit::gen_quotient(cons, nullptr, chunk_cost, per_unit);
        }
        if (p->jit.quotient.units.empty() && (p->n_constraints || p->n_groups)) { p->jit.state = -1; p->jit.error = "code generation failed"; continue; }
        todo.push_back(p);
    }
    if (todo.empty()) return 0;
    std::vector<std::string> sources;
    for (PwProver* p : todo) {
        for (auto& u : p->jit.quotient.units) sources.push_back(u.source);
        for (auto& u : p->jit.perm.units) sources.push_back(u.source);
    }
    std::string err;
    std::vector<jit::ProgramPtr> progs = jit::compile_all(sources, &err);
    if (progs.empty() && todo.size() > 1) {
        for (PwProver* p : todo) { PwProver* one[1] = {p}; uint32_t lh = 40; p->jit.state = 0; p->jit.quotient = {}; p->jit.perm = {}; (void)specialise_provers(one, 1, &lh, true); }
        return 0;
    }
    int n_dev = 0;
    const bool have_device = hipGetDeviceCount(&n_dev) == hipSuccess && n_dev > 0;
    if (!have_device) (void)hipGetLastError();
    size_t k = 0;
    for (PwProver* p : todo) {
        if (progs.empty()) { p->jit.state = -1; p->jit.error = err; p->jit.quotient = {}; p->jit.perm = {}; continue; }
        p->jit.quotient_prog.assign(progs.begin() + (long)k, progs.begin() + (long)(k + p->jit.quotient.units.size()));
        k += p->jit.quotient.units.size();
        p->jit.perm_prog.assign(progs.begin() + (long)k, progs.begin() + (long)(k + p->jit.perm.units.size()));
        k += p->jit.perm.units.size();
        for (auto& u : p->jit.quotient.units) { u.source.clear(); u.source.shrink_to_fit(); }
        for (auto& u : p->jit.perm.units) { u.source.clear(); u.source.shrink_to_fit(); }
        p->jit.state = 1;
        if (have_device) {
            std::string e2;
            bool ok = true;
            for (size_t u = 0; u < p->jit.quotient.units.size() && ok; ++u) ok = jit::kernel(*p->jit.quotient_prog[u], p->jit.quotient.units[u].kernel.c_str(), &e2) != nullptr;
            for (size_t u = 0; u < p->jit.perm.units.size() && ok; ++u) ok = jit::kernel(*p->jit.perm_prog[u], p->jit.perm.units[u].kernel.c_str(), &e2) != nullptr;
            if (!ok) {
                (void)hipGetLastError();
                p->jit.state = -1;
                p->jit.error = "the compiled kernels do not load on this device: " + e2;
                p->jit.quotient_prog.clear(); p->jit.perm_prog.clear(); p->jit.quotient = {}; p->jit.perm = {};
            }
        }
    }
    return 0;
}

size_t jit_part_bytes(const PwProver* p, size_t H, size_t q_rows) {
    if (p->jit.state != 1) return 0;
    const size_t a = (size_t)(p->jit.perm.n_chunks ? p->jit.perm.n_chunks : (p->logup ? 1 : 0)) * 16 * H;
    const size_t b = (size_t)(p->jit.quotient.n_chunks ? p->jit.quotient.n_chunks : 1) * 16 * q_rows;
    return a > b ? a : b;
}

int quotient_parts_jit(PwProver* p, const uint32_t* T, const uint32_t* Pm, size_t rows, const bb::Ext* d_apow, bb::Ext al, const bb::Ext* d_blpow,
                       uint32_t* part, uint32_t* n_chunks) {
    const jit::Generated& g = p->jit.quotient;
    uint64_t n64 = rows;
    const uint32_t* pub = p->d_pub;
    void* args[] = {(void*)&T, (void*)&Pm, (void*)&n64, (void*)&d_apow, (void*)&al, (void*)&d_blpow, (void*)&part, (void*)&pub};
    ScopedKernelTimer t(Pm ? "quotient_logup_jit_kernel" : "quotient_jit_kernel");
    const int rc = launch_units(g, p->jit.quotient_prog, rows, args);
    if (n_chunks) *n_chunks = g.n_chunks;
    return rc;
}

uint32_t quotient_units_jit(const PwProver* p) { return (uint32_t)p->jit.quotient.units.size(); }
void quotient_unit_groups(const PwProver* p, uint32_t u, uint32_t* g0, uint32_t* g1) {
    *g0 = p->jit.quotient.units[u].g0;
    *g1 = p->jit.quotient.units[u].g1;
}
uint32_t quotient_max_unit_perm_cols(const PwProver* p) {
    uint32_t w = 0;
    for (const auto& u : p->jit.quotient.units) w = std::max(w, 4 * (u.g1 - u.g0));
    return w;
}
int quotient_unit_jit(PwProver* p, uint32_t u, const uint32_t* T, const uint32_t* Pm, size_t rows, const bb::Ext* d_apow, bb::Ext al,
                      const bb::Ext* d_blpow, uint32_t* part) {
    const jit::Generated& g = p->jit.quotient;
    uint64_t n64 = rows;
    const uint32_t* pub = p->d_pub;
    void* args[] = {(void*)&T, (void*)&Pm, (void*)&n64, (void*)&d_apow, (void*)&al, (void*)&d_blpow, (void*)&part, (void*)&pub};
    ScopedKernelTimer t(Pm ? "quotient_logup_jit_kernel" : "quotient_jit_kernel");
    return launch_unit(g, p->jit.quotient_prog, u, rows, args);
}

int quotient_eval_jit(PwProver* p, const uint32_t* lde, size_t N, const bb::Ext* d_apow, uint32_t zinv_even, uint32_t zinv_odd, uint32_t* q) {
    PW_TRY_INT(p->qpart.ensure(jit_part_bytes(p, N / 2, N)));
    uint32_t* part = p->qpart.as<uint32_t>();
    uint32_t n_chunks = 0;
    PW_TRY_INT(quotient_parts_jit(p, lde, nullptr, N, d_apow, bb::ext_zero(), nullptr, part, &n_chunks));
    return quotient_combine(part, n_chunks, N, zinv_even, zinv_odd, q);
}

int quotient_eval_logup_jit(PwProver* p, const uint32_t* lde, const uint32_t* plde, size_t N, int logN, const bb::Ext* d_apow, bb::Ext al,
                            const bb::Ext* d_blpow, bb::Ext S, uint32_t zval_even, uint32_t zval_odd, uint32_t* q) {
    PW_TRY_INT(p->qpart.ensure(jit_part_bytes(p, N / 2, N)));
    uint32_t* part = p->qpart.as<uint32_t>();
    uint32_t n_chunks = 0;
    PW_TRY_INT(quotient_parts_jit(p, lde, plde, N, d_apow, al, d_blpow, part, &n_chunks));
    const uint32_t G = p->n_groups;
    return quotient_logup_tail(part, n_chunks, plde + (size_t)(4 * G) * N, plde + (size_t)(4 * G + 4) * N, N, logN, d_apow + p->n_constraints + G, S,
                               zval_even, zval_odd, q);
}

int logup_perm_trace_jit(PwProver* p, const uint32_t* trace, size_t H, bb::Ext al, const bb::Ext* d_blpow, uint32_t* perm, bb::Ext* d_rowsum,
                         bb::Ext* d_block_totals) {
    const jit::Generated& g = p->jit.perm;
    const uint32_t G = p->n_groups;
    PW_TRY_INT(p->qpart.ensure((size_t)(g.n_chunks ? g.n_chunks : 1) * 4 * H * 4));
    uint32_t* part = p->qpart.as<uint32_t>();
    uint64_t h64 = H;
    void* args[] = {(void*)&trace, (void*)&h64, (void*)&al, (void*)&d_blpow, (void*)&perm, (void*)&part};
    {
        ScopedKernelTimer t("logup_perm_jit_kernel");
        const int rc = launch_units(g, p->jit.perm_prog, H, args);
        if (rc) return rc;
    }
    int rc = logup_rowsum_combine(part, g.n_chunks, H, d_rowsum, perm + (size_t)(4 * G + 4) * H);
    if (rc) return rc;
    return logup_scan(d_rowsum, H, d_block_totals, perm + (size_t)(4 * G) * H);
}

}

extern "C" int pw_prover_specialise(PwProver* p) {
    if (!p) return -1;
    PwProver* ps[1] = {p};
    (void)pw::specialise_provers(ps, 1, nullptr, true);
    return p->jit.state == 1 ? 0 : 1;
}

extern "C" size_t pw_provers_specialise(PwProver* const* ps, size_t n) {
    if (!ps || !n) return 0;
    (void)pw::specialise_provers(ps, n, nullptr, true);
    size_t ok = 0;
    for (size_t i = 0; i < n; ++i) ok += ps[i] && ps[i]->jit.state == 1;
    return ok;
}

extern "C" int pw_prover_specialised(const PwProver* p, size_t* n_kernels, size_t* code_bytes, size_t* n_chunks) {
    if (!p) return -1;
    size_t k = 0, b = 0, c = 0;
    if (p->jit.state == 1) {
        k = p->jit.quotient_prog.size() + p->jit.perm_prog.size();
        for (auto& pr : p->jit.quotient_prog) b += pw::jit::code_bytes(*pr);
        for (auto& pr : p->jit.perm_prog) b += pw::jit::code_bytes(*pr);
        c = p->jit.quotient.n_chunks + p->jit.perm.n_chunks;
    }
    if (n_kernels) *n_kernels = k;
    if (code_bytes) *code_bytes = b;
    if (n_chunks) *n_chunks = c;
    return p->jit.state;
}

extern "C" void pw_jit_cache_stats(uint64_t* units_compiled, uint64_t* units_from_disk) { pw::jit::cache_stats(units_compiled, units_from_disk); }
```

powdr_amd/csrc/prover_stages.hpp:

```cpp
#pragma once
#include "prover_stream.hpp"
#include "logup_groups.hpp"

#include <algorithm>
#include <cstdlib>
#include <cstring>
#include <vector>

namespace pw {

#define PW_STRY(x) do { const int _rc = (x); if (_rc) return _rc; } while (0)

struct AirShape {
    uint32_t W, nc, n_int, n_g, log_h;
    uint32_t Wp;
    uint32_t M;
    uint32_t Wf, W1;
    uint32_t rf, Wr, Wg;
    uint32_t K1, K;
    size_t H, N;
    int logN;
};

inline AirShape air_shape(const PwProver* p, uint32_t log_h, bool logup) {
    AirShape s{};
    s.W = p->width; s.nc = p->n_constraints; s.log_h = log_h;
    s.n_int = logup ? p->n_inter : 0; s.n_g = logup ? p->n_groups : 0; s.Wp = logup ? 4 * (s.n_g + 1) : 0;
    s.M = s.nc + (logup ? s.n_g + 3 : 0);
    s.Wf = p->pre_width; s.W1 = s.W + s.Wf;
    s.rf = p->row_flags; s.Wr = p->row_cols; s.Wg = (s.rf & kRowsNext) ? s.W1 : 0;
    s.K1 = s.W1 + s.Wp + 8;
    s.K = s.K1 + s.Wp + s.Wg;
    s.H = (size_t)1 << log_h; s.N = 2 * s.H; s.logN = (int)log_h + 1;
    return s;
}

struct AirMode {
    int b;
    bool eat;
};

inline size_t dot_scratch_words(const AirShape& s) { return 2 * (size_t)std::max({s.W1, s.Wp, 8u}) * div_up(s.H, 8192); }

inline streamed::Ctx stream_ctx(PwProver* p, const AirShape& s, const CommitLayout& L) {
    return streamed::Ctx{p, s.log_h, L.b, L.perm_panels, s.H, s.N, L.m, s.W, s.Wp};
}

inline ConstraintProgram constraint_program(const PwProver* p, uint32_t nc) {
    ConstraintProgram c{p->d_bytecode, p->d_spans, nc, p->is_xbc};
    if (p->n_public) { c.d_pub = p->d_pub; c.pub_base = p->pub_base; }
    return c;
}

inline LogupProgram logup_program(const PwProver* p, const AirShape& s) {
    return s.Wp ? LogupProgram{p->d_inter, s.n_int, p->d_ixspans, p->d_icode, p->d_gstarts, s.n_g, p->d_iforms} : LogupProgram{};
}

struct BufferPlan {
    size_t coef = 0, lde = 0, digests = 0, tcoef = 0, fscale = 0, perm = 0, plde = 0, q = 0, qpart = 0, qcoef = 0, qlde = 0, gbuf = 0,
           ext_arena = 0, misc = 0;
    size_t total() const { return coef + lde + digests + tcoef + fscale + perm + plde + q + qpart + qcoef + qlde + gbuf + ext_arena + misc; }
    BufferPlan commit_part() const { BufferPlan C; C.coef = coef; C.lde = lde; C.digests = digests; C.tcoef = tcoef; C.fscale = fscale; return C; }
};

inline void plan_stage_buffers(const PwProver* p, const AirShape& s, AirMode m, CommitLayout& L, BufferPlan& B) {
    const size_t H = s.H, N = s.N;
    const bool lg = s.Wp != 0;
    const int b = m.b;
    L.H = H; L.N = N; L.b = b; L.m = N >> b;
    L.panel_cols = lde_panel_cols(H, b ? 8 : std::max<size_t>(s.W, s.Wp));
    B.coef = L.panel_cols * H * 4;
    L.perm_panels = b && lg && specialised(p) && !getenv("POWDR_STREAM_NO_PANELS");
    if (!b) B.lde = ((size_t)s.W1 + s.Wr) * N * 4;
    else if (L.perm_panels) B.lde = std::max<size_t>(std::max(s.W, s.Wp), (size_t)s.W + quotient_max_unit_perm_cols(p)) * L.m * 4;
    else B.lde = (size_t)(s.W + s.Wp) * L.m * 4;
    if (b || s.log_h >= kDeepComboMinLogHeight) B.gbuf = (size_t)24 * H * 4;
    if (lg) {
        B.perm = (size_t)(s.Wp + kJitExtraPermCols) * H * 4;
        B.plde = b ? (size_t)8 * N * 4 : (size_t)(s.Wp + kJitExtraPermCols) * N * 4;
    }
    B.q = 4 * N * 4;
    const size_t q_rows = L.m;
    if (!lg) {
        const uint32_t chunks = quotient_chunks(q_rows, s.nc);
        if (chunks > 1) B.qpart = (size_t)chunks * 4 * q_rows * 4;
    }
    if (b) B.qpart += 4 * L.m * 4;
    B.qpart = std::max(B.qpart, jit_part_bytes(p, H, q_rows));
    if (b && m.eat && lg) {
        B.perm = std::max(B.perm, (size_t)s.W * H * 4);
        B.lde = std::max(B.lde, (size_t)(s.Wp + kJitExtraPermCols) * H * 4);
    }
    B.qcoef = 8 * H * 4;
    B.qlde = 8 * N * 4;
}

inline int apply_plan(PwProver* p, const BufferPlan& B) {
    const struct { DeviceBuf* buf; size_t bytes; } all[] = {
        {&p->coef, B.coef}, {&p->lde, B.lde}, {&p->digests, B.digests}, {&p->tcoef, B.tcoef}, {&p->fscale, B.fscale}, {&p->perm, B.perm},
        {&p->plde, B.plde}, {&p->q, B.q}, {&p->qpart, B.qpart}, {&p->qcoef, B.qcoef}, {&p->qlde, B.qlde}, {&p->ext_arena, B.ext_arena},
        {&p->misc, B.misc}, {&p->gbuf, B.gbuf}};
    for (const auto& e : all)
        if (e.bytes) PW_STRY(e.buf->ensure(e.bytes));
    return 0;
}

struct AirBufs {
    const uint32_t* trace;
    const uint32_t* values;
    uint32_t* tcoef;
    bb::Ext* apow;
    bb::Ext* blpow;
    bb::Ext* weights;
    bb::Ext* weights2;
    bb::Ext* rowsum;
    bb::Ext* scratch;
};

inline int logup_stage(PwProver* p, const AirShape& s, AirMode m, const CommitLayout& L, const AirBufs& B, bb::Ext al, const uint32_t* s_words[4]) {
    const size_t H = s.H;
    const bool jit = specialised(p);
    uint32_t* d_perm = p->perm.as<uint32_t>();
    uint32_t* d_pval = m.eat ? p->lde.as<uint32_t>() : d_perm;
    if (jit) PW_STRY(logup_perm_trace_jit(p, B.values, H, al, B.blpow, d_pval, B.rowsum, B.rowsum + H));
    else PW_STRY(logup_perm_trace(B.values, H, logup_program(p, s), al, B.blpow, d_pval, B.rowsum, B.rowsum + H));
    const uint32_t* phi_last = d_pval + ((size_t)(4 * s.n_g) * H + (H - 1));
    if (!m.b) {
        PW_STRY(lde_matrix(p, L, s.log_h, d_perm, s.Wp + (jit ? kJitExtraPermCols : 0u), p->plde.as<uint32_t>()));
        for (int k = 0; k < 4; ++k) s_words[k] = phi_last + (size_t)k * H;
        return 0;
    }
    if (!jit) PW_STRY(ext_to_cols(B.rowsum, H, d_pval + (size_t)(4 * s.n_g + 4) * H));
    PW_STRY(lde_matrix(p, L, s.log_h, d_pval + (size_t)(4 * s.n_g) * H, 8, p->plde.as<uint32_t>()));
    uint32_t* d_save = p->gbuf.as<uint32_t>();
    for (int k = 0; k < 4; ++k) {
        PW_HIP_TRY(hipMemcpyAsync(d_save + k, phi_last + (size_t)k * H, 4, hipMemcpyDeviceToDevice, stream()));
        s_words[k] = d_save + k;
    }
    if (m.eat) {
        PW_HIP_TRY(hipMemcpyAsync(B.tcoef, d_perm, (size_t)s.W * H * 4, hipMemcpyDeviceToDevice, stream()));
        PW_STRY(intt_dif(d_pval, d_perm, H, H, s.Wp, (int)s.log_h));
    } else PW_STRY(intt_dif(d_perm, d_perm, H, H, s.Wp, (int)s.log_h));
    return 0;
}

inline int quotient_stage(PwProver* p, const AirShape& s, AirMode m, const CommitLayout& L, const AirBufs& B, bb::Ext al, bb::Ext S) {
    const bool lg = s.Wp != 0, jit = specialised(p);
    const uint32_t one = bb::R_MOD_P;
    uint32_t sH = bb::to_monty(field::kCosetShift);
    for (uint32_t i = 0; i < s.log_h; ++i) sH = bb::sqr(sH);
    const uint32_t zv_even = bb::sub(sH, one), zv_odd = bb::sub(bb::neg(sH), one);
    const ConstraintProgram prog = constraint_program(p, s.nc);
    uint32_t* d_lde = p->lde.as<uint32_t>();
    uint32_t* d_plde = p->plde.as<uint32_t>();
    uint32_t* d_q = p->q.as<uint32_t>();
    if (m.b) {
        PW_STRY(streamed::quotient_sums(stream_ctx(p, s, L), jit, lg, s.nc, prog, logup_program(p, s), B.tcoef, p->perm.as<uint32_t>(), B.apow, al,
                                        B.blpow, S, s.logN, d_q));
        if (lg) PW_STRY(quotient_logup_tail(d_q, 1, d_plde, d_plde + 4 * s.N, s.N, s.logN, B.apow + s.nc + s.n_g, S, zv_even, zv_odd, d_q));
        else PW_STRY(quotient_combine(d_q, 1, s.N, bb::inv(zv_even), bb::inv(zv_odd), d_q));
    } else if (lg && jit)
        PW_STRY(quotient_eval_logup_jit(p, d_lde, d_plde, s.N, s.logN, B.apow, al, B.blpow, S, zv_even, zv_odd, d_q));
    else if (lg)
        PW_STRY(quotient_eval_logup(d_lde, d_plde, s.N, s.logN, prog, logup_program(p, s), B.apow, al, B.blpow, S, zv_even, zv_odd, d_q));
    else if (jit && s.nc)
        PW_STRY(quotient_eval_jit(p, d_lde, s.N, B.apow, bb::inv(zv_even), bb::inv(zv_odd), d_q));
    else
        PW_STRY(quotient_eval(d_lde, s.N, prog, B.apow, bb::inv(zv_even), bb::inv(zv_odd), d_q, p->qpart.as<uint32_t>(), quotient_chunks(s.N, s.nc)));
    PW_STRY(intt_dif(d_q, d_q, s.N, s.N, 4, s.logN));
    PW_STRY(quotient_split(d_q, s.H, (int)s.log_h, p->qcoef.as<uint32_t>()));
    return coset_lde_from_coeffs(p->qcoef.as<uint32_t>(), p->qlde.as<uint32_t>(), s.H, s.N, 8, (int)s.log_h);
}

template <class AfterPiece>
inline int open_stage(PwProver* p, const AirShape& s, AirMode m, const AirBufs& B, bb::Ext zeta, bb::Ext gzeta, bb::Ext* o, const uint32_t* slice_at,
                      uint32_t n_slices, AfterPiece&& after_piece) {
    const int log_h = (int)s.log_h;
    const size_t H = s.H;
    auto open_perm = [&]() -> int {
        for (uint32_t i = 0; i < n_slices; ++i) {
            const uint32_t c0 = slice_at[i], c1 = slice_at[i + 1];
            if (c1 > c0)
                PW_STRY(ext_dot_columns2(p->perm.as<uint32_t>() + (size_t)c0 * H, H, c1 - c0, H, B.weights, B.weights2, o + s.W1 + c0, o + s.K1 + c0, B.scratch));
            PW_STRY(after_piece());
        }
        return 0;
    };
    if (!m.eat) {
        PW_STRY(barycentric_weights(zeta, log_h, B.weights));
        if (s.Wg) {
            PW_STRY(barycentric_weights(gzeta, log_h, B.weights2));
            PW_STRY(ext_dot_columns2(B.values, H, s.W1, H, B.weights, B.weights2, o, o + s.K1 + s.Wp, B.scratch));
        } else
            PW_STRY(ext_dot_columns(B.values, H, s.W1, H, B.weights, o, B.scratch));
        PW_STRY(after_piece());
    }
    if (s.Wp && !m.b) {
        if (!s.Wg) PW_STRY(barycentric_weights(gzeta, log_h, B.weights2));
        PW_STRY(open_perm());
    }
    PW_STRY(zeta_weights(zeta, log_h, B.weights));
    if (m.eat) {
        PW_STRY(ext_dot_columns(B.tcoef, H, s.W, H, B.weights, o, B.scratch));
        PW_STRY(after_piece());
    }
    if (s.Wp && m.b) {
        PW_STRY(zeta_weights(gzeta, log_h, B.weights2));
        PW_STRY(open_perm());
    }
    PW_STRY(ext_dot_columns(p->qcoef.as<uint32_t>(), H, 8, H, B.weights, o + s.W1 + s.Wp, B.scratch));
    return after_piece();
}

template <class Sums>
inline int deep_stage(PwProver* p, const AirShape& s, AirMode m, const CommitLayout& L, const AirBufs& B, const bb::Ext* d_gpow, bb::Ext gamma,
                      Sums&& sums, const bb::Ext& sum1, const bb::Ext& sum2, bb::Ext zeta, bb::Ext gzeta, bb::Ext* out) {
    const bool lg = s.Wp != 0;
    uint32_t* d_lde = p->lde.as<uint32_t>();
    uint32_t* d_plde = p->plde.as<uint32_t>();
    uint32_t* d_qlde = p->qlde.as<uint32_t>();
    if (m.b)
        return streamed::deep_from_coefficients(stream_ctx(p, s, L), lg, B.tcoef, p->perm.as<uint32_t>(), d_qlde, s.logN, d_gpow, sums, sum1, sum2, zeta,
                                                gzeta, out);
    if (s.Wg) {
        sums();
        return deep_quotient_two_point(d_lde, s.W1, lg ? d_plde : nullptr, s.Wp, d_qlde, s.N, s.logN, d_gpow, bb::ext_pow(gamma, s.K1 + s.Wp), sum1, sum2,
                                       zeta, gzeta, out);
    }
    if (s.log_h >= kDeepComboMinLogHeight && !s.Wf && !getenv("POWDR_DEEP_DIRECT") && !((uintptr_t)B.trace & 7)) {
        uint32_t* d_gev = p->gbuf.as<uint32_t>();
        uint32_t* d_glde = d_gev + 8 * s.H;
        PW_STRY(ext_lincomb(B.trace, s.W, p->perm.as<uint32_t>(), s.Wp, s.H, d_gpow, lg ? s.K1 : 0u, d_gev));
        PW_STRY(lde_matrix(p, L, s.log_h, d_gev, lg ? 8u : 4u, d_glde));
        sums();
        return deep_from_combo(d_glde, d_qlde, s.N, s.logN, d_gpow + s.W + s.Wp, sum1, sum2, zeta, gzeta, lg ? 1 : 0, out);
    }
    sums();
    if (lg) return deep_quotient_logup(d_lde, s.W1, d_plde, s.Wp, d_qlde, s.N, s.logN, d_gpow, sum1, sum2, zeta, gzeta, out);
// ... 53 lines not shown
```

powdr_amd/csrc/prover_state.hpp:

```cpp
#pragma once
#include "prover_internal.hpp"
#include "jit_codegen.hpp"
#include "jit.hpp"
#include "../../include/powdr_prover.h"

#include <cstring>
#include <vector>

namespace pw {

constexpr uint32_t kMagic = 0x31535750u;
constexpr uint32_t kMagic2 = 0x32535750u;
constexpr uint32_t kMagic3 = 0x33535750u;
constexpr uint32_t kMagic4 = 0x34535750u;
constexpr uint32_t kMagic5 = 0x35535750u;
constexpr uint32_t kMagic6 = 0x36535750u;

struct Challenger {
    uint32_t st[16];
    std::vector<uint32_t> in, out;
    Challenger() { memset(st, 0, sizeof st); }
    void duplex() {
        for (size_t i = 0; i < in.size(); ++i) st[i] = in[i];
        in.clear();
        p2::permute(st, poseidon2_params_host());
        out.assign(st, st + 8);
    }
    void observe(uint32_t m) { out.clear(); in.push_back(m); if (in.size() == 8) duplex(); }
    void observe_canonical(uint32_t c) { observe(bb::to_monty(c)); }
    void observe_words(const uint32_t* w, size_t n) { for (size_t i = 0; i < n; ++i) observe(w[i]); }
    void observe_ext(const bb::Ext& e) { observe_words(e.c, 4); }
    uint32_t sample() { if (!in.empty() || out.empty()) duplex(); uint32_t v = out.back(); out.pop_back(); return v; }
    bb::Ext sample_ext() { bb::Ext e; for (int i = 0; i < 4; ++i) e.c[i] = sample(); return e; }
    uint32_t sample_bits(int b) { return bb::from_monty(sample()) & ((1u << b) - 1u); }
};

struct DeviceBuf {
    void* p = nullptr;
    size_t bytes = 0;
    int device = -1;
    int ensure(size_t need) {
        int dev = 0;
        hipError_t e = hipGetDevice(&dev);
        if (e != hipSuccess) return (int)e;
        if (p && dev == device && need <= bytes) return 0;
        if (p) (void)hipFree(p);
        p = nullptr; bytes = 0;
        e = hipMalloc(&p, need);
        if (e != hipSuccess) return (int)e;
        bytes = need;
        device = dev;
        return 0;
    }
    void release() { if (p) (void)hipFree(p); p = nullptr; bytes = 0; }
    template <class T> T* as() { return reinterpret_cast<T*>(p); }
    DeviceBuf() = default;
    DeviceBuf(const DeviceBuf&) = delete;
    DeviceBuf& operator=(const DeviceBuf&) = delete;
    ~DeviceBuf() { release(); }
};

int gather_records(const uint32_t* arena, const uint64_t* d_offsets, uint32_t words_per_record, uint32_t n, uint32_t* out);

}

struct PwProver {
    PwStarkConfig cfg;
    uint32_t width;
    std::vector<uint32_t> h_spans;
    uint32_t n_constraints;
    uint32_t* d_bytecode = nullptr;
    uint32_t* d_spans = nullptr;
    bool is_xbc = false;
    int max_degree = 0;
    bool logup = false;
    uint32_t n_inter = 0, n_groups = 0, max_args = 0;
    uint32_t* d_gstarts = nullptr;
    pw::LogupInteraction* d_inter = nullptr;
    uint32_t* d_ixspans = nullptr;
    uint32_t* d_icode = nullptr;
    pw::SmallForm* d_iforms = nullptr;
    pw::DeviceBuf perm, plde;
    pw::DeviceBuf bus_order;
    std::vector<uint32_t> h_bus_order, h_bus_ids, h_bus_starts;
    bool has_bus_seed = false;
    uint32_t bus_seed[8] = {0};
    const uint32_t* committed_trace = nullptr;
    uint32_t committed_log_h = 0;
    uint32_t committed_root[8] = {0};
    int committed_b = 0;
    pw::DeviceBuf coef, lde, digests, q, qcoef, qlde, ext_arena, misc;
    pw::DeviceBuf qpart;
    pw::DeviceBuf tcoef, fscale, gbuf;
    struct OpenedMailbox {
        static constexpr int kEvents = 8;
        bb::Ext* host = nullptr;
        bb::Ext* dev = nullptr;
        size_t cap = 0;
        int device = -1;
        hipEvent_t ev[kEvents] = {};
        int n_events = 0;
    } opened_mb;
    std::vector<uint32_t> proof;
    uint32_t pre_width = 0, pre_log_h = 0;
    uint32_t pre_root[8] = {0};
    pw::DeviceBuf pre_vals, pre_lde, pre_tree;
    bool transition = false;
    uint32_t row_flags = 0, row_cols = 0;
    std::vector<uint32_t> h_next_cols;
    uint32_t* d_next_cols = nullptr;
    pw::DeviceBuf row_vals;
    uint32_t n_public = 0, pub_base = 0xffffffffu;
    bool pub_set = false;
    std::vector<uint32_t> h_pub;
    uint32_t* d_pub = nullptr;
    std::vector<uint32_t> h_xcode, h_xspans, h_icode, h_ixspans, h_gstarts;
    std::vector<pw::LogupInteraction> h_inter;
    struct Specialised {
        int state = 0;
        pw::jit::Generated quotient, perm;
        std::vector<pw::jit::ProgramPtr> quotient_prog, perm_prog;
        std::string error;
    } jit;
};

namespace pw {
struct CommitLayout {
    size_t H, N, tree_words, fri_words, n_trees, panel_cols;
    int b = 0;
    size_t m = 0;
    bool perm_panels = false;
};
constexpr uint32_t kDeepComboMinLogHeight = 16;
int lde_matrix(PwProver* p, const CommitLayout& L, uint32_t log_h, const uint32_t* m, uint32_t cols, uint32_t* out);
size_t lde_panel_cols(size_t H, size_t widest);

size_t proof_plan_bytes(const PwProver* p, uint32_t log_h, int b, bool consume = false);
int ensure_proof_buffers(PwProver* p, uint32_t log_h, int b, CommitLayout& L, bool consume = false);
inline uint32_t stream_min_log_height() {
    const char* e = getenv("POWDR_STREAM_MIN_LOG_HEIGHT");
    return e ? (uint32_t)atoi(e) : 16u;
}
bool device_room(size_t held, size_t* avail);
size_t device_budget();

int specialise_provers(PwProver* const* ps, size_t n, const uint32_t* log_heights, bool force);
pw::jit::Generated generate_sources(const PwProver* p, int which, uint32_t chunk_cost, uint32_t chunks_per_unit);
inline bool specialised(const PwProver* p) { return p->jit.state == 1; }
int quotient_eval_jit(PwProver* p, const uint32_t* lde, size_t N, const bb::Ext* d_apow, uint32_t zinv_even, uint32_t zinv_odd, uint32_t* q);
int quotient_parts_jit(PwProver* p, const uint32_t* T, const uint32_t* Pm, size_t rows, const bb::Ext* d_apow, bb::Ext al, const bb::Ext* d_blpow,
                       uint32_t* part, uint32_t* n_chunks);
uint32_t quotient_units_jit(const PwProver* p);
void quotient_unit_groups(const PwProver* p, uint32_t u, uint32_t* g0, uint32_t* g1);
int quotient_unit_jit(PwProver* p, uint32_t u, const uint32_t* T, const uint32_t* Pm, size_t rows, const bb::Ext* d_apow, bb::Ext al,
                      const bb::Ext* d_blpow, uint32_t* part);
uint32_t quotient_max_unit_perm_cols(const PwProver* p);
size_t jit_part_bytes(const PwProver* p, size_t H, size_t q_rows);
int quotient_eval_logup_jit(PwProver* p, const uint32_t* lde, const uint32_t* plde, size_t N, int logN, const bb::Ext* d_apow, bb::Ext al,
                            const bb::Ext* d_blpow, bb::Ext S, uint32_t zval_even, uint32_t zval_odd, uint32_t* q);
int logup_perm_trace_jit(PwProver* p, const uint32_t* trace, size_t H, bb::Ext al, const bb::Ext* d_blpow, uint32_t* perm, bb::Ext* d_rowsum,
                         bb::Ext* d_block_totals);
constexpr uint32_t kJitExtraPermCols = 4;
}
```

powdr_amd/prover.py:

```python
from __future__ import annotations

import ctypes as C

import numpy as np

from . import abi

lib = abi.lib


class PwStarkConfig(C.Structure):
    _fields_ = [("num_queries", C.c_uint32), ("pow_bits", C.c_uint32)]


PROVER_SYMBOLS = ["pw_prover_check_constraints", "pw_verify", "pw_prover_create", "pw_prover_create_logup", "pw_verify_logup", "pw_prover_trace_root", "pw_prover_set_bus_seed", "pw_prover_logup_path", "pw_prove_airs", "pw_verify_airs", "pw_prove_segment", "pw_verify_segment", "pw_commitment_digest", "pw_logup_group_starts", "pw_prover_width", "pw_prover_reserve", "pw_prover_stream_log_blocks", "pw_prover_max_constraint_degree", "pw_prover_destroy", "pw_prover_prove", "pw_prover_prove_consuming", "pw_prover_stream_log_blocks_consuming", "pw_trace_from_coefficients", "pw_prover_device_bytes",
                  "pw_lde_batch", "pw_lde_fused", "pw_lde_subcoset", "pw_merkle_commit", "pw_poseidon2_permute_host",
                  "pw_set_poseidon2_constants", "pw_get_poseidon2_constants", "pw_prover_specialise", "pw_prover_specialised", "pw_jit_compile_check", "pw_jit_cache_stats", "pw_jit_generated_source",
                  "pw_prove_segments_multi", "pw_multi_last_merge", "pw_assign_units",
                  "pw_prove_segment_consuming", "pw_segment_last_modes", "pw_segment_last_plan", "pw_set_device_budget", "pw_get_device_budget", "pw_provers_specialise",
                  "pw_segment_context_bytes", "pw_segment_stream_plan", "pw_segment_last_plan_tables",
                  "pw_prover_create_preprocessed", "pw_prover_preprocessed_root", "pw_prover_preprocessed_width", "pw_verify_segment_preprocessed",
                  "pw_prover_create_transition", "pw_prover_row_flags", "pw_verify_segment_transition",
                  "pw_prover_create_public", "pw_prover_n_public", "pw_prover_set_public_values", "pw_verify_segment_public",
                  "pw_segment_proof_public_values", "pw_verify_segment_chain", "pw_public_programs_check",
                  "pw_check_segment_buses", "pw_bus_check_scratch_bytes", "pw_bus_check_peak_bytes", "pw_bus_check_last_stats",
                  "pw_poseidon2_compress_trace"]

lib.pw_prover_create.restype = C.c_void_p
lib.pw_prover_create.argtypes = [C.POINTER(PwStarkConfig), C.c_uint32, C.c_void_p, C.c_size_t, C.c_void_p, C.c_size_t]
lib.pw_prover_create_logup.restype = C.c_void_p
lib.pw_prover_create_logup.argtypes = [C.POINTER(PwStarkConfig), C.c_uint32, C.c_void_p, C.c_size_t, C.c_void_p, C.c_size_t,
                                       C.c_void_p, C.c_size_t, C.c_void_p, C.c_size_t, C.c_void_p, C.c_size_t]
lib.pw_prover_destroy.argtypes = [C.c_void_p]
lib.pw_prover_create_preprocessed.restype = C.c_void_p
lib.pw_prover_create_preprocessed.argtypes = [C.POINTER(PwStarkConfig), C.c_uint32, C.c_uint32, C.c_uint32, C.c_void_p, C.c_void_p, C.c_size_t,
                                              C.c_void_p, C.c_size_t, C.c_void_p, C.c_size_t, C.c_void_p, C.c_size_t, C.c_void_p, C.c_size_t]
lib.pw_prover_preprocessed_root.restype = C.c_int
lib.pw_prover_preprocessed_root.argtypes = [C.c_void_p, C.c_void_p]
lib.pw_prover_preprocessed_width.restype = C.c_uint32
lib.pw_prover_preprocessed_width.argtypes = [C.c_void_p]
lib.pw_prover_create_transition.restype = C.c_void_p
lib.pw_prover_create_transition.argtypes = lib.pw_prover_create_preprocessed.argtypes
lib.pw_prover_row_flags.restype = C.c_uint32
lib.pw_prover_row_flags.argtypes = [C.c_void_p]
lib.pw_prover_create_public.restype = C.c_void_p
lib.pw_prover_create_public.argtypes = lib.pw_prover_create_preprocessed.argtypes[:5] + [C.c_uint32] + lib.pw_prover_create_preprocessed.argtypes[5:]
lib.pw_prover_n_public.restype = C.c_uint32
lib.pw_prover_n_public.argtypes = [C.c_void_p]
lib.pw_prover_set_public_values.restype = C.c_int
lib.pw_prover_set_public_values.argtypes = [C.c_void_p, C.c_void_p, C.c_size_t]
lib.pw_prover_prove.restype = C.c_int
lib.pw_prover_prove.argtypes = [C.c_void_p, C.c_void_p, C.c_uint32, C.POINTER(C.POINTER(C.c_uint32)), C.POINTER(C.c_size_t)]
lib.pw_prover_check_constraints.restype = C.c_int
lib.pw_prover_check_constraints.argtypes = [C.c_void_p, C.c_void_p, C.c_uint32, C.POINTER(C.c_uint64), C.POINTER(C.c_uint64),
                                            C.POINTER(C.c_uint32)]
lib.pw_prover_device_bytes.restype = C.c_size_t
lib.pw_prover_device_bytes.argtypes = [C.c_void_p]
lib.pw_lde_batch.restype = C.c_int
lib.pw_lde_batch.argtypes = [C.c_void_p, C.c_uint32, C.c_uint32, C.c_void_p, C.c_void_p]
lib.pw_lde_fused.restype = C.c_int
lib.pw_lde_fused.argtypes = [C.c_void_p, C.c_uint32, C.c_uint32, C.c_void_p, C.c_void_p]
lib.pw_prover_prove_consuming.restype = C.c_int
lib.pw_prover_prove_consuming.argtypes = lib.pw_prover_prove.argtypes
lib.pw_prover_stream_log_blocks_consuming.restype = C.c_int
lib.pw_prover_stream_log_blocks_consuming.argtypes = [C.c_void_p, C.c_uint32]
lib.pw_trace_from_coefficients.restype = C.c_int
lib.pw_trace_from_coefficients.argtypes = [C.c_void_p, C.c_uint32, C.c_uint32, C.c_void_p]
lib.pw_lde_subcoset.restype = C.c_int
lib.pw_lde_subcoset.argtypes = [C.c_void_p, C.c_uint32, C.c_uint32, C.c_uint32, C.c_uint32, C.c_void_p, C.c_void_p]
lib.pw_segment_last_modes.restype = C.c_size_t
lib.pw_segment_last_modes.argtypes = [C.c_void_p, C.c_size_t]
lib.pw_segment_context_bytes.restype = C.c_size_t
lib.pw_segment_context_bytes.argtypes = []
lib.pw_segment_stream_plan.restype = C.c_size_t
lib.pw_segment_stream_plan.argtypes = [C.c_size_t, C.c_void_p, C.c_void_p, C.c_void_p, C.c_size_t, C.c_size_t, C.c_void_p]
lib.pw_segment_last_plan_tables.restype = C.c_size_t
lib.pw_segment_last_plan_tables.argtypes = [C.c_void_p, C.c_void_p, C.c_void_p, C.c_size_t]
lib.pw_set_device_budget.restype = None
lib.pw_set_device_budget.argtypes = [C.c_size_t]
lib.pw_get_device_budget.restype = C.c_size_t
lib.pw_merkle_commit.restype = C.c_int
lib.pw_merkle_commit.argtypes = [C.c_void_p, C.c_size_t, C.c_uint32, C.c_void_p]
lib.pw_poseidon2_permute_host.argtypes = [C.c_void_p]


def _vp(a):
    return a.ctypes.data_as(C.c_void_p)


def _interaction_tables(interactions):
    if interactions is None:
        return (None, 0, None, 0, None, 0), []
    it = np.ascontiguousarray(interactions[0], dtype=np.uint32).reshape(-1, 3)
    isp = np.ascontiguousarray(interactions[1], dtype=np.uint32).reshape(-1, 2)
    ibc = np.ascontiguousarray(interactions[2], dtype=np.uint32)
    return (_vp(it), len(it), _vp(isp), len(isp), _vp(ibc), len(ibc)), [it, isp, ibc]


lib.pw_verify.restype = C.c_int
lib.pw_verify.argtypes = [C.POINTER(PwStarkConfig), C.c_uint32, C.c_uint32, C.c_void_p, C.c_size_t, C.c_void_p, C.c_size_t,
# ... 391 lines not shown
    lk = (PwChainLink * max(len(links), 1))(*[PwChainLink(*[int(x) for x in l]) for l in links])
    cfg = PwStarkConfig(num_queries, pow_bits)
    where = C.c_size_t(0)
    rc = int(lib.pw_verify_segment_chain(C.byref(cfg), segs, n, lk, len(links), C.byref(where)))
    return rc, int(where.value)


def public_programs_check(width: int, cons_bytecode, cons_spans, n_public: int, interactions=None, pre_width: int = 0):
    bc = np.ascontiguousarray(cons_bytecode, dtype=np.uint32)
    sp = np.ascontiguousarray(cons_spans, dtype=np.uint32).reshape(-1, 2)
    tables, _ = _interaction_tables(interactions)
    deg, rf, nx, ns = C.c_int(), C.c_uint32(), C.c_size_t(), C.c_size_t()
    args = (width, pre_width, n_public, _vp(bc), len(bc), _vp(sp), len(sp), *tables, C.byref(deg), C.byref(rf))
    if lib.pw_public_programs_check(*args, None, 0, C.byref(nx), None, 0, C.byref(ns)) != 0:
        return None
    xbc, src = np.zeros(max(nx.value, 1), np.uint32), C.create_string_buffer(ns.value + 1)
    lib.pw_public_programs_check(*args, _vp(xbc), nx.value, C.byref(nx), src, ns.value + 1, C.byref(ns))
    return dict(max_degree=deg.value, row_flags=rf.value, xbc=xbc[:nx.value].copy(), source=src.value.decode())


def verify_airs(descs, proofs, num_queries: int = 100, pow_bits: int = 0, shared_bus_seed: bool = False, check_balance: bool = False):
    n = len(descs)
    recs, keep = _air_descriptions(descs)
    prs = [np.ascontiguousarray(p, dtype=np.uint32) for p in proofs]
    ptrs = (C.c_void_p * max(n, 1))(*[p.ctypes.data for p in prs])
    lens = (C.c_size_t * max(n, 1))(*[len(p) for p in prs])
    cfg = PwStarkConfig(num_queries, pow_bits)
    total = np.zeros(4, np.uint32)
    rc = int(lib.pw_verify_airs(C.byref(cfg), recs, n, ptrs, lens, int(shared_bus_seed), int(check_balance), _vp(total)))
    return rc, total


def poseidon2_host(state) -> np.ndarray:
    s = np.ascontiguousarray(state, dtype=np.uint32).copy()
    lib.pw_poseidon2_permute_host(s.ctypes.data_as(C.c_void_p))
    return s


lib.pw_set_poseidon2_constants.restype = C.c_int
lib.pw_set_poseidon2_constants.argtypes = [C.c_void_p, C.c_void_p]
lib.pw_get_poseidon2_constants.restype = None
lib.pw_get_poseidon2_constants.argtypes = [C.c_void_p, C.c_void_p, C.c_void_p]


def jit_compile_check(width: int, cons_bytecode, cons_spans, interactions=None) -> dict:
    vp = lambda a: a.ctypes.data_as(C.c_void_p)
    bc = np.ascontiguousarray(cons_bytecode, dtype=np.uint32)
    sp = np.ascontiguousarray(cons_spans, dtype=np.uint32).reshape(-1, 2)
    k, b, c = C.c_size_t(), C.c_size_t(), C.c_size_t()
    err = C.create_string_buffer(4096)
    f = lib.pw_jit_compile_check
    f.restype = C.c_int
    f.argtypes = [C.c_uint32, C.c_void_p, C.c_size_t, C.c_void_p, C.c_size_t, C.c_void_p, C.c_size_t, C.c_void_p, C.c_size_t, C.c_void_p, C.c_size_t,
                  C.POINTER(C.c_size_t), C.POINTER(C.c_size_t), C.POINTER(C.c_size_t), C.c_char_p, C.c_size_t]
    tables, _ = _interaction_tables(interactions)
    rc = f(width, vp(bc), len(bc), vp(sp), len(sp), *tables, C.byref(k), C.byref(b), C.byref(c), err, 4096)
    return dict(rc=int(rc), kernels=k.value, code_bytes=b.value, chunks=c.value, error=err.value.decode(errors="replace"))


def jit_generated_sources(width: int, cons_bytecode, cons_spans, interactions=None, which: int = 0, chunk_cost: int = 0, chunks_per_unit: int = 0):
    vp = lambda a: a.ctypes.data_as(C.c_void_p)
    bc = np.ascontiguousarray(cons_bytecode, dtype=np.uint32)
    sp = np.ascontiguousarray(cons_spans, dtype=np.uint32).reshape(-1, 2)
    f = lib.pw_jit_generated_source
    f.restype = C.c_size_t
    f.argtypes = [C.c_uint32, C.c_void_p, C.c_size_t, C.c_void_p, C.c_size_t, C.c_void_p, C.c_size_t, C.c_void_p, C.c_size_t, C.c_void_p, C.c_size_t,
                  C.c_int, C.c_uint32, C.c_uint32, C.c_size_t, C.c_char_p, C.c_size_t, C.c_char_p, C.c_size_t, C.POINTER(C.c_uint32),
                  C.POINTER(C.c_uint32), C.POINTER(C.c_uint32)]
    tables, _ = _interaction_tables(interactions)
    units, total = [], C.c_uint32()
    while True:
        first, n, name = C.c_uint32(), C.c_uint32(), C.create_string_buffer(64)
        size = f(width, vp(bc), len(bc), vp(sp), len(sp), *tables, which, chunk_cost, chunks_per_unit, len(units), None, 0, name, 64, C.byref(first), C.byref(n),
                 C.byref(total))
        if size == 0:
            break
        buf = C.create_string_buffer(size + 1)
        f(width, vp(bc), len(bc), vp(sp), len(sp), *tables, which, chunk_cost, chunks_per_unit, len(units), buf, size + 1, name, 64, C.byref(first), C.byref(n),
          C.byref(total))
        units.append(dict(source=buf.value.decode(), kernel=name.value.decode(), first_chunk=first.value, n_chunks=n.value))
    return units, total.value


def jit_cache_stats() -> dict:
    lib.pw_jit_cache_stats.restype = None
    lib.pw_jit_cache_stats.argtypes = [C.POINTER(C.c_uint64), C.POINTER(C.c_uint64)]
    a, b = C.c_uint64(), C.c_uint64()
    lib.pw_jit_cache_stats(C.byref(a), C.byref(b))
    return dict(compiled=a.value, from_disk=b.value)


_SEGMENT_PROVE_FN = C.CFUNCTYPE(C.c_int, C.c_void_p, C.c_size_t, C.c_size_t, C.c_int, C.POINTER(C.c_uint32))
lib.pw_prove_segments_multi.restype = C.c_int
lib.pw_prove_segments_multi.argtypes = [C.POINTER(C.c_int), C.c_size_t, C.POINTER(C.c_uint64), C.c_size_t, _SEGMENT_PROVE_FN, C.c_void_p,
                                        C.c_void_p, C.c_void_p]
lib.pw_multi_last_merge.restype = C.c_int
lib.pw_assign_units.restype = C.c_size_t
lib.pw_assign_units.argtypes = [C.POINTER(C.c_uint64), C.c_size_t, C.c_size_t, C.c_void_p]


def assign_units(cells, n_workers: int) -> np.ndarray:
    n = len(cells)
    out = np.zeros(n, np.uint32)
    arr = (C.c_uint64 * max(n, 1))(*[int(c) for c in cells])
    assert lib.pw_assign_units(arr, n, n_workers, out.ctypes.data_as(C.c_void_p)) == n
    return out


def prove_segments_multi(devices, segment_cells, prove_segment):
    n = len(segment_cells)
    errors = []

    def cb(_user, segment, worker, device, out):
        try:
            c = np.asarray(prove_segment(int(segment), int(worker), int(device)), dtype=np.uint32).reshape(8)
            for i in range(8):
                out[i] = int(c[i])
            return 0
        except Exception as e:
            errors.append(e)
            return 1

    fn = _SEGMENT_PROVE_FN(cb)
    devs = (C.c_int * len(devices))(*[int(d) for d in devices])
    cells = (C.c_uint64 * max(n, 1))(*[int(c) for c in segment_cells])
    commitments = np.zeros((n, 8), np.uint32)
    owner = np.zeros(n, np.uint32)
    rc = lib.pw_prove_segments_multi(devs, len(devices), cells, n, fn, None, commitments.ctypes.data_as(C.c_void_p), owner.ctypes.data_as(C.c_void_p))
    if errors:
        raise errors[0]
    abi.check(rc, "pw_prove_segments_multi")
    return commitments, owner, int(lib.pw_multi_last_merge())


def set_poseidon2_constants(ext_rc=None, int_rc=None) -> None:
    if ext_rc is None:
        rc = lib.pw_set_poseidon2_constants(None, None)
    else:
        e = np.ascontiguousarray(ext_rc, dtype=np.uint32).reshape(8, 16)
        i = np.ascontiguousarray(int_rc, dtype=np.uint32).reshape(13)
        rc = lib.pw_set_poseidon2_constants(e.ctypes.data_as(C.c_void_p), i.ctypes.data_as(C.c_void_p))
    if rc:
        raise ValueError("round constants must be canonical field elements")


def poseidon2_constants():
    e, i, d = np.zeros((8, 16), np.uint32), np.zeros(13, np.uint32), np.zeros(16, np.uint32)
    lib.pw_get_poseidon2_constants(e.ctypes.data_as(C.c_void_p), i.ctypes.data_as(C.c_void_p), d.ctypes.data_as(C.c_void_p))
    return e, i, d


class Prover:

    def __init__(self, width: int, cons_bytecode, cons_spans, num_queries: int = 100, pow_bits: int = 0, interactions=None,
                 preprocessed=None, transition: bool = False, n_public: int = 0):
        bc = np.ascontiguousarray(cons_bytecode, dtype=np.uint32)
        sp = np.ascontiguousarray(cons_spans, dtype=np.uint32).reshape(-1, 2)
        cfg = PwStarkConfig(num_queries, pow_bits)
        self.width = width
        self.pre_width = 0
        self.n_public = int(n_public)
        tables, _ = _interaction_tables(interactions)
        if n_public:
            t, pw_, lh = preprocessed if preprocessed is not None else (None, 0, 0)
            if t is not None:
                assert t.numel() == pw_ << lh, "the fixed matrix must hold pre_width x 2^log_height words"
# ... 110 lines not shown
```

rust/powdr-hip/src/ffi.rs:

```rust
#![allow(non_camel_case_types, clippy::too_many_arguments)]

use core::ffi::{c_char, c_int, c_uint, c_void};

pub type PowdrFp = u32;

#[repr(C)]
#[derive(Clone, Copy, Debug)]
pub struct OriginalAir {
    pub width: i32,
    pub height: i32,
    pub buffer: *const PowdrFp,
    pub row_block_size: i32,
}
#[repr(C)]
#[derive(Clone, Copy, Debug)]
pub struct Subst {
    pub air_index: i32,
    pub col: i32,
    pub row: i32,
    pub apc_col: i32,
}
#[repr(C)]
#[derive(Clone, Copy)]
pub struct ExprSpan {
// ... 336 lines not shown
    pub fn pw_prover_prove_consuming(p: *mut PwProver, d_trace: *mut u32, log_height: u32, proof_words: *mut *const u32,
                                     n_words: *mut usize) -> c_int;
    pub fn pw_prover_stream_log_blocks_consuming(p: *const PwProver, log_height: u32) -> c_int;
    pub fn pw_trace_from_coefficients(d_coeffs: *mut u32, width: u32, log_height: u32, d_scratch: *mut u32) -> c_int;
    pub fn pw_prover_check_constraints(p: *mut PwProver, d_trace: *const u32, log_height: u32, n_violations: *mut u64,
                                       first_row: *mut u64, first_constraint: *mut u32) -> c_int;
    pub fn pw_check_segment_buses(airs: *const PwSegmentAir, n_airs: usize, buses: *const u32, n_buses: usize, seed: u64,
                                  table_bytes: usize, flags: u32, summaries: *mut PwBusSummary, summary_cap: usize,
                                  n_summaries: *mut usize, tuples: *mut PwBusTuple, tuple_cap: usize, n_tuples: *mut usize) -> c_int;
    pub fn pw_bus_check_scratch_bytes() -> usize;
    pub fn pw_bus_check_peak_bytes() -> usize;
    pub fn pw_program_frequencies(airs: *const PwSegmentAir, n_airs: usize, bus: u32, pc_base: u32, pc_step: u32, d_program: *const u32,
                                  log_h: u32, d_freq_out: *mut u32, n_foreign: *mut u64, first_foreign: *mut PwBusTuple) -> c_int;
    pub fn pw_memory_boundary_trace(airs: *const PwSegmentAir, n_airs: usize, bus: u32, table_bytes: usize, d_trace_out: *mut u32,
                                    cap_log_height: u32, log_height: *mut u32, n_locations: *mut u64, status: *mut u32) -> c_int;
    pub fn pw_system_traces_scratch_bytes() -> usize;
    pub fn pw_system_traces_peak_bytes() -> usize;
    pub fn pw_system_traces_last_stats(out: *mut PwSystemTraceStats);
    pub fn pw_memory_boundary_set_start_slots(log_slots: u32) -> c_int;
    pub fn pw_poseidon2_compress_trace(airs: *const PwSegmentAir, n_airs: usize, bus: u32, table_bytes: usize, start_log_slots: u32,
                                       d_trace_out: *mut u32, cap_log_height: u32, log_height: *mut u32, n_rows: *mut u64,
                                       status: *mut u32) -> c_int;
    pub fn pw_verify(cfg: *const PwStarkConfig, width: u32, log_height: u32, cons_bytecode: *const u32, bytecode_len: usize,
                     cons_spans: *const u32, n_constraints: usize, proof_words: *const u32, n_words: usize) -> c_int;
    pub fn pw_verify_logup(cfg: *const PwStarkConfig, width: u32, log_height: u32, cons_bytecode: *const u32,
                           bytecode_len: usize, cons_spans: *const u32, n_constraints: usize, interactions: *const u32,
                           n_interactions: usize, inter_spans: *const u32, n_inter_spans: usize,
                           inter_bytecode: *const u32, inter_bytecode_len: usize, expected_bus_seed: *const u32,
                           proof_words: *const u32, n_words: usize, cumulative_sum: *mut u32, trace_root: *mut u32) -> c_int;
    pub fn pw_logup_group_starts(interactions: *const u32, n_interactions: usize, inter_spans: *const u32,
                                 n_inter_spans: usize, inter_bytecode: *const u32, inter_bytecode_len: usize,
                                 out: *mut u32, cap: usize) -> usize;
    pub fn pw_prove_segment(airs: *const PwSegmentAir, n_airs: usize, logup: c_int, proof_words: *mut *const u32,
                            n_words: *mut usize) -> c_int;
    pub fn pw_prove_segment_consuming(airs: *const PwSegmentAir, n_airs: usize, logup: c_int, proof_words: *mut *const u32,
                                      n_words: *mut usize) -> c_int;
    pub fn pw_provers_specialise(provers: *const *mut PwProver, n: usize) -> usize;
    pub fn pw_segment_last_modes(out: *mut u32, cap: usize) -> usize;
    pub fn pw_segment_last_plan(resident_bytes: *mut usize, planned_bytes: *mut usize, available_bytes: *mut usize);
    pub fn pw_segment_context_bytes() -> usize;
    pub fn pw_set_device_budget(bytes: usize);
    pub fn pw_get_device_budget() -> usize;
    pub fn pw_verify_segment(cfg: *const PwStarkConfig, airs: *const PwAirDescription, n_airs: usize, logup: c_int,
                             proof_words: *const u32, n_words: usize, check_balance: c_int, total_sum4: *mut u32) -> c_int;
    pub fn pw_verify_segment_preprocessed(cfg: *const PwStarkConfig, airs: *const PwAirDescription, pre: *const PwAirPreprocessed,
                                          n_airs: usize, logup: c_int, proof_words: *const u32, n_words: usize, check_balance: c_int,
                                          total_sum4: *mut u32) -> c_int;
    pub fn pw_verify_segment_transition(cfg: *const PwStarkConfig, airs: *const PwAirDescription, pre: *const PwAirPreprocessed,
                                        n_airs: usize, logup: c_int, proof_words: *const u32, n_words: usize, check_balance: c_int,
                                        total_sum4: *mut u32) -> c_int;
    pub fn pw_verify_segment_public(cfg: *const PwStarkConfig, airs: *const PwAirDescription, pre: *const PwAirPreprocessed,
                                    pub_: *const PwAirPublic, n_airs: usize, logup: c_int, proof_words: *const u32, n_words: usize,
                                    check_balance: c_int, total_sum4: *mut u32) -> c_int;
    pub fn pw_segment_proof_public_values(airs: *const PwAirDescription, pub_: *const PwAirPublic, n_airs: usize, proof_words: *const u32,
                                          n_words: usize, air: usize, out: *mut u32, cap: usize) -> usize;
    pub fn pw_verify_segment_chain(cfg: *const PwStarkConfig, segments: *const PwChainSegment, n_segments: usize, links: *const PwChainLink,
                                   n_links: usize, where_: *mut usize) -> c_int;
    pub fn pw_prove_airs(airs: *const PwSegmentAir, n_airs: usize, shared_bus_seed: c_int, n_workers: c_uint,
                         proofs: *mut *const u32, n_words: *mut usize, bus_seed8: *mut u32) -> c_int;
    pub fn pw_verify_airs(cfg: *const PwStarkConfig, airs: *const PwAirDescription, n_airs: usize,
                          proofs: *const *const u32, n_words: *const usize, shared_bus_seed: c_int,
                          check_balance: c_int, total_sum4: *mut u32) -> c_int;
    pub fn pw_commitment_digest(roots8: *const u32, n: usize, digest8: *mut u32);
    pub fn pw_prover_reserve(p: *mut PwProver, log_height: u32) -> c_int;
    pub fn pw_prover_stream_log_blocks(p: *const PwProver, log_height: u32) -> c_int;
    pub fn pw_prover_max_constraint_degree(p: *const PwProver) -> c_int;
    pub fn pw_prover_width(p: *const PwProver) -> u32;
    pub fn pw_prover_device_bytes(p: *const PwProver) -> usize;
    pub fn pw_lde_batch(d_trace: *const u32, width: u32, log_height: u32, d_coeffs: *mut u32, d_lde: *mut u32) -> c_int;
    pub fn pw_lde_fused(d_trace: *const u32, width: u32, log_height: u32, d_tmp: *mut u32, d_lde: *mut u32) -> c_int;
    pub fn pw_lde_subcoset(d_coeffs: *const u32, width: u32, log_height: u32, log_blocks: u32, r: u32, d_scale: *mut u32, d_out: *mut u32) -> c_int;
    pub fn pw_merkle_commit(d_matrix: *const u32, height: usize, width: u32, d_digests: *mut u32) -> c_int;
    pub fn pw_prover_specialise(p: *mut PwProver) -> c_int;
    pub fn pw_prover_specialised(p: *const PwProver, n_kernels: *mut usize, code_bytes: *mut usize, n_chunks: *mut usize) -> c_int;
    pub fn pw_prove_segments_multi(devices: *const c_int, n_workers: usize, segment_cells: *const u64, n_segments: usize,
                                   prove: PwSegmentProveFn, user: *mut c_void, commitments: *mut u32, worker_of_segment: *mut u32) -> c_int;
    pub fn pw_multi_last_merge() -> c_int;
    pub fn pw_assign_units(cells: *const u64, n_units: usize, n_workers: usize, worker_of_unit: *mut u32) -> usize;
    pub fn pw_jit_generated_source(width: u32, cons_bytecode: *const u32, bytecode_len: usize, cons_spans: *const u32, n_constraints: usize,
                                   interactions: *const u32, n_interactions: usize, inter_spans: *const u32, n_inter_spans: usize,
                                   inter_bytecode: *const u32, inter_bytecode_len: usize, which: c_int, chunk_cost: u32, chunks_per_unit: u32,
                                   unit: usize, buf: *mut c_char, cap: usize, kernel_name: *mut c_char, name_cap: usize, first_chunk: *mut u32,
                                   n_chunks: *mut u32, total_chunks: *mut u32) -> usize;
    pub fn pw_jit_cache_stats(units_compiled: *mut u64, units_from_disk: *mut u64);
    pub fn pw_jit_compile_check(width: u32, cons_bytecode: *const u32, bytecode_len: usize, cons_spans: *const u32, n_constraints: usize,
                                interactions: *const u32, n_interactions: usize, inter_spans: *const u32, n_inter_spans: usize,
                                inter_bytecode: *const u32, inter_bytecode_len: usize, n_kernels: *mut usize, code_bytes: *mut usize,
                                n_chunks: *mut usize, err: *mut c_char, err_cap: usize) -> c_int;
    pub fn pw_poseidon2_permute_host(state16: *mut u32);
    pub fn pw_set_poseidon2_constants(ext_rc: *const u32, int_rc: *const u32) -> c_int;
    pub fn pw_get_poseidon2_constants(ext_rc: *mut u32, int_rc: *mut u32, diag: *mut u32);
}

extern "C" {
    pub fn hipMalloc(ptr: *mut *mut c_void, bytes: usize) -> c_int;
    pub fn hipFree(ptr: *mut c_void) -> c_int;
    pub fn hipMemcpy(dst: *mut c_void, src: *const c_void, bytes: usize, kind: c_int) -> c_int;
    pub fn hipMemset(dst: *mut c_void, value: c_int, bytes: usize) -> c_int;
    pub fn hipDeviceSynchronize() -> c_int;
    pub fn hipSetDevice(device: c_int) -> c_int;
}
pub const HIP_MEMCPY_HOST_TO_DEVICE: c_int = 1;
pub const HIP_MEMCPY_DEVICE_TO_HOST: c_int = 2;
```

Before: 7.135 billion.

## Fold quotient weights into per-group LogUp denominator coefficient tables

Adds a small per-proof device table that premultiplies each LogUp group's quotient weight into its denominator seed and beta-power coefficients, for groups of one or two interactions. The JIT quotient kernel then reads these folded coefficients and accumulates the weighted terms directly, dropping an extension multiply per group and the separate numerator/denominator combination. It also lowers the chunk cost estimate for such groups, and the JIT compiler now uses helper processes even when only one is requested. The cost is an extra small kernel launch, an extra buffer, more kernel arguments and table loads per row.

```diff
diff --git a/include/powdr_prover.h b/include/powdr_prover.h
--- a/include/powdr_prover.h
+++ b/include/powdr_prover.h
@@ -218,6 +218,9 @@
                                const uint32_t* inter_bytecode, size_t inter_bytecode_len, int which, uint32_t chunk_cost, uint32_t chunks_per_unit,
                                size_t unit, char* buf, size_t cap, char* kernel_name, size_t name_cap, uint32_t* first_chunk, uint32_t* n_chunks,
                                uint32_t* total_chunks);
+size_t pw_quotient_fold_table_host(const uint32_t* interactions, size_t n_interactions, const uint32_t* inter_spans, size_t n_inter_spans,
+                                   const uint32_t* inter_bytecode, size_t inter_bytecode_len, const uint32_t* apow_groups,
+                                   const uint32_t* alpha_l, const uint32_t* blpow, uint32_t* out, size_t cap_words, uint32_t* row_words);
 void pw_jit_cache_stats(uint64_t* units_compiled, uint64_t* units_from_disk);
 int pw_jit_compile_check(uint32_t width, const uint32_t* cons_bytecode, size_t bytecode_len, const uint32_t* cons_spans, size_t n_constraints,
                          const uint32_t* interactions, size_t n_interactions, const uint32_t* inter_spans, size_t n_inter_spans,
diff --git a/powdr_amd/csrc/host/jit.cpp b/powdr_amd/csrc/host/jit.cpp
--- a/powdr_amd/csrc/host/jit.cpp
+++ b/powdr_amd/csrc/host/jit.cpp
@@ -366,7 +366,7 @@
             if (n_procs > todo.size()) n_procs = (unsigned)todo.size();
             std::vector<std::vector<char>> code(todo.size());
             bool compiled = false;
-            const std::string helper = n_procs > 1 ? helper_path() : std::string();
+            const std::string helper = helper_path();
             std::string e;
             if (!helper.empty() && compile_with_helpers(helper, sources, todo, n_procs, code, compiled, &e)) {
                 if (!compiled) { if (err) *err = e; return {}; }
diff --git a/powdr_amd/csrc/host/jit_codegen.cpp b/powdr_amd/csrc/host/jit_codegen.cpp
--- a/powdr_amd/csrc/host/jit_codegen.cpp
+++ b/powdr_amd/csrc/host/jit_codegen.cpp
@@ -1,6 +1,7 @@
 #include "../jit_codegen.hpp"
 #include "../xbc.hpp"
 
+#include <algorithm>
 #include <cstdio>
 #include <unordered_map>
 
@@ -94,8 +95,15 @@
 
 struct Chunk { uint32_t c0, c1, g0, g1; };
 
-uint32_t group_cost(const LogupView& lg, uint32_t g) {
-    uint32_t cost = 150;
+uint32_t fold_row_words_of(const LogupView& lg) {
+    uint32_t max_args = 0;
+    for (uint32_t i = 0; i < lg.n_inter; ++i) max_args = std::max(max_args, lg.inter[i].n_args);
+    return 8u + 4u * max_args;
+}
+
+uint32_t group_cost(const LogupView& lg, uint32_t g, bool folded) {
+    const uint32_t n = lg.gstarts[g + 1] - lg.gstarts[g];
+    uint32_t cost = folded && n == 1 ? 75 : folded && n == 2 ? 95 : 150;
     for (uint32_t i = lg.gstarts[g]; i < lg.gstarts[g + 1]; ++i) {
         const LogupInteraction& it = lg.inter[i];
         cost += 60 + 14 * it.n_args;
@@ -104,19 +112,25 @@
     return cost;
 }
 
-bool emit_member(Emitter& e, const LogupView& lg, uint32_t i, uint32_t g, uint32_t k, std::string& m) {
+bool emit_member(Emitter& e, const LogupView& lg, uint32_t i, uint32_t g, uint32_t k, std::string& m, const char* fold_w = nullptr,
+                 uint32_t fold_off = 0) {
     const LogupInteraction& it = lg.inter[i];
     const uint32_t* sp = lg.exprs.spans + 2 * (size_t)it.first_span;
     if (!e.expr(lg.exprs.code + 2 * (size_t)sp[0], sp[1], m)) return false;
     std::vector<std::string> args(it.n_args);
     for (uint32_t j = 0; j < it.n_args; ++j)
         if (!e.expr(lg.exprs.code + 2 * (size_t)sp[2 + 2 * j], sp[3 + 2 * j], args[j])) return false;
-    char b[160];
+    char b[224];
     if (it.n_args) {
         snprintf(b, sizeof b, "const uint32_t a%u_%u[%u] = {", g, k, it.n_args);
         e.out += b;
         for (uint32_t j = 0; j < it.n_args; ++j) e.out += (j ? ", " : "") + args[j];
-        snprintf(b, sizeof b, "};\nconst Ext d%u_%u = pwj::denominator<%u>(sd, %uu, blpow, a%u_%u);\n", g, k, it.n_args, it.bus_monty, g, k);
+        if (fold_w) snprintf(b, sizeof b, "};\nconst Ext e%u = pwj::denominator_folded<%u>(fold, %uu, %s, al, %uu, blpow, a%u_%u);\n", g, it.n_args, fold_off, fold_w,
+                             it.bus_monty, g, k);
+        else snprintf(b, sizeof b, "};\nconst Ext d%u_%u = pwj::denominator<%u>(sd, %uu, blpow, a%u_%u);\n", g, k, it.n_args, it.bus_monty, g, k);
+        e.out += b;
+    } else if (fold_w) {
+        snprintf(b, sizeof b, "const Ext e%u = pwj::denominator_folded0(fold, %uu, %s, al, %uu);\n", g, fold_off, fold_w, it.bus_monty);
         e.out += b;
     } else {
         snprintf(b, sizeof b, "const Ext d%u_%u = pwj::denominator0(sd, %uu);\n", g, k, it.bus_monty);
@@ -125,7 +139,7 @@
     return true;
 }
 
-std::vector<Chunk> cut(const XbcView* cons, const LogupView* lg, uint32_t chunk_cost, size_t& total_cost) {
+std::vector<Chunk> cut(const XbcView* cons, const LogupView* lg, uint32_t chunk_cost, size_t& total_cost, bool folded) {
     std::vector<Chunk> chunks;
     total_cost = 0;
     if (cons) {
@@ -141,7 +155,7 @@
     if (lg) {
         uint32_t g0 = 0, acc = 0;
         for (uint32_t g = 0; g < lg->n_groups; ++g) {
-            const uint32_t cost = group_cost(*lg, g);
+            const uint32_t cost = group_cost(*lg, g, folded);
             if (acc && acc + cost > chunk_cost) { chunks.push_back({0, 0, g0, g}); g0 = g; acc = 0; }
             acc += cost;
             total_cost += cost;
@@ -189,8 +203,9 @@
 
 Generated gen_quotient(const XbcView& cons, const LogupView* lg, uint32_t chunk_cost, uint32_t chunks_per_unit) {
     size_t total = 0;
-    const std::vector<Chunk> chunks = cut(&cons, lg, chunk_cost, total);
+    const std::vector<Chunk> chunks = cut(&cons, lg, chunk_cost, total, true);
     const uint32_t nc = cons.n;
+    const uint32_t fold_words = lg ? fold_row_words_of(*lg) : 0;
     bool has_pub = false;
     for (uint32_t c = 0; c < cons.n && !has_pub; ++c)
         for (uint32_t i = cons.spans[2 * c], end = i + cons.spans[2 * c + 1]; i < end && !has_pub; ++i) has_pub = cons.code[2 * (size_t)i] >= xbc::SET_PUB;
@@ -214,12 +229,21 @@
                                       "pwj::ld(Pm + (size_t)%uu * N, j4)}};\n", g, 4 * g, 4 * g + 1, 4 * g + 2, 4 * g + 3);
                 s += b;
                 std::vector<std::string> m(n);
-                for (uint32_t k = 0; k < n; ++k) if (!emit_member(e, *lg, i0 + k, g, k, m[k])) return false;
-                const std::string G = std::to_string(g);
+                const std::string G = std::to_string(g), w = "apow[" + std::to_string(nc + g) + "]";
+                const bool folded = n == 1 || n == 2;
+                for (uint32_t k = 0; k < n; ++k)
+                    if (!emit_member(e, *lg, i0 + k, g, k, m[k], folded && k == 0 ? w.c_str() : nullptr, g * fold_words)) return false;
+                if (n == 1) {
+                    s += "wide.fma(q" + G + ", e" + G + ");\nwide.fma_base(" + w + ", bb::neg(" + m[0] + "));\n";
+                    continue;
+                }
+                if (n == 2) {
+                    s += "const Ext x" + G + " = pwj::sub_scaled(bb::ext_mul(q" + G + ", e" + G + "), " + w + ", " + m[0] + ");\n";
+                    s += "wide.fma(x" + G + ", d" + G + "_1);\nwide.fma_base(e" + G + ", bb::neg(" + m[1] + "));\n";
+                    continue;
+                }
                 if (n == 0) {
                     s += "const Ext term" + G + " = q" + G + ";\n";
-                } else if (n == 1) {
-                    s += "Ext term" + G + " = bb::ext_mul(q" + G + ", d" + G + "_0);\nterm" + G + ".c[0] = bb::sub(term" + G + ".c[0], " + m[0] + ");\n";
                 } else {
                     s += "Ext den" + G + " = bb::ext_mul(d" + G + "_0, d" + G + "_1);\n";
                     s += "Ext num" + G + " = pwj::scale2(d" + G + "_1, " + m[0] + ", d" + G + "_0, " + m[1] + ");\n";
@@ -240,20 +264,23 @@
         s += b;
         return true;
     };
-    Generated g = assemble(chunks, chunks_per_unit, "pwj_quotient_",
-                           has_pub ? "(const uint32_t* __restrict__ T, const uint32_t* __restrict__ Pm, size_t N, const Ext* __restrict__ apow, Ext al, "
-                                     "const Ext* __restrict__ blpow, uint32_t* __restrict__ part, const uint32_t* __restrict__ pub)"
-                                   : "(const uint32_t* __restrict__ T, const uint32_t* __restrict__ Pm, size_t N, const Ext* __restrict__ apow, Ext al, "
-                                     "const Ext* __restrict__ blpow, uint32_t* __restrict__ part)",
+    std::string signature = "(const uint32_t* __restrict__ T, const uint32_t* __restrict__ Pm, size_t N, const Ext* __restrict__ apow, Ext al, "
+                            "const Ext* __restrict__ blpow, uint32_t* __restrict__ part";
+    if (has_pub) signature += ", const uint32_t* __restrict__ pub";
+    if (lg) signature += ", const uint32_t* __restrict__ fold = nullptr";
+    signature += ")";
+    Generated g = assemble(chunks, chunks_per_unit, "pwj_quotient_", signature.c_str(),
                            "const uint32_t j = blockIdx.x * 256u + threadIdx.x;\nif (j >= N) return;\nconst uint32_t j4 = j * 4u;\n", "", body);
     g.est_instructions = total;
     g.has_pub = has_pub;
+    g.has_fold = lg != nullptr;
+    g.fold_row_words = fold_words;
     return g;
 }
 
 Generated gen_logup_perm(const LogupView& lg, uint32_t chunk_cost, uint32_t chunks_per_unit) {
     size_t total = 0;
-    const std::vector<Chunk> chunks = cut(nullptr, &lg, chunk_cost, total);
+    const std::vector<Chunk> chunks = cut(nullptr, &lg, chunk_cost, total, false);
     constexpr uint32_t kBatch = 4;
     auto body = [&](const Chunk& ch, uint32_t id, std::string& s) -> bool {
         Emitter e(s, "T");
diff --git a/powdr_amd/csrc/jit_codegen.hpp b/powdr_amd/csrc/jit_codegen.hpp
--- a/powdr_amd/csrc/jit_codegen.hpp
+++ b/powdr_amd/csrc/jit_codegen.hpp
@@ -31,6 +31,8 @@
     uint32_t n_chunks = 0;
     size_t est_instructions = 0;
     bool has_pub = false;
+    bool has_fold = false;
+    uint32_t fold_row_words = 0;
 };
 
 Generated gen_quotient(const XbcView& cons, const LogupView* lg, uint32_t chunk_cost, uint32_t chunks_per_unit);
diff --git a/powdr_amd/csrc/jit_device.hpp b/powdr_amd/csrc/jit_device.hpp
--- a/powdr_amd/csrc/jit_device.hpp
+++ b/powdr_amd/csrc/jit_device.hpp
@@ -28,10 +28,17 @@
     uint32_t pending;
     __device__ __forceinline__ DenominatorAcc(const DenominatorSeeds& sd, uint32_t bus_monty)
         : T{(int64_t)bb::centred(bb::add(sd.al0, bus_monty)) * (int64_t)bb::R_MOD_P, sd.s[1], sd.s[2], sd.s[3]}, pending(0) {}
+    __device__ __forceinline__ explicit DenominatorAcc(const int64_t (&seed)[4]) : T{seed[0], seed[1], seed[2], seed[3]}, pending(0) {}
     __device__ __forceinline__ void reduce() {
 #pragma unroll
         for (int k = 0; k < 4; ++k) T[k] = bb::smul_uniform(bb::smont(T[k]), (int32_t)bb::R_MOD_P);
         pending = 0;
+    }
+    __device__ __forceinline__ void add_centred(uint32_t a, const int32_t (&c)[4]) {
+        if (pending == 2) reduce();
+#pragma unroll
+        for (int k = 0; k < 4; ++k) T[k] = bb::swide_mad_uniform(T[k], (int32_t)a, c[k]);
+        ++pending;
     }
     __device__ __forceinline__ void add(uint32_t a, const Ext& b) {
         if (pending == 2) reduce();
@@ -60,6 +67,61 @@
 __device__ __forceinline__ Ext denominator0(const DenominatorSeeds& sd, uint32_t bus_monty) {
     DenominatorAcc acc(sd, bus_monty);
     return acc.result();
+}
+
+PW_HD uint32_t fold_row_words(uint32_t max_args) { return 8u + 4u * max_args; }
+PW_HD void fold_seeds(const Ext& w, const Ext& al, uint32_t bus_monty, uint32_t* row) {
+    Ext t = al;
+    t.c[0] = bb::add(t.c[0], bus_monty);
+    const Ext e = bb::ext_mul(w, t);
+    for (int k = 0; k < 4; ++k) {
+        const int64_t s = (int64_t)bb::centred(e.c[k]) * (int64_t)bb::R_MOD_P;
+        row[2 * k] = (uint32_t)(uint64_t)s;
+        row[2 * k + 1] = (uint32_t)((uint64_t)s >> 32);
+    }
+}
+PW_HD void fold_coefficient(const Ext& w, const Ext& b, uint32_t* row4) {
+    const Ext e = bb::ext_mul(w, b);
+    for (int k = 0; k < 4; ++k) row4[k] = (uint32_t)bb::centred(e.c[k]);
+}
+PW_HD void fold_row(const Ext& w, const Ext& al, uint32_t bus_monty, uint32_t n_args, const Ext* blpow, uint32_t* row) {
+    fold_seeds(w, al, bus_monty, row);
+    for (uint32_t j = 0; j < n_args; ++j) fold_coefficient(w, blpow[j + 1], row + 8 + 4 * j);
+}
+__device__ __forceinline__ Ext denominator_of_row(const uint32_t* __restrict__ row, const uint32_t* a, int n_args) {
+    int64_t seed[4];
+#pragma unroll
+    for (int k = 0; k < 4; ++k) seed[k] = (int64_t)(((uint64_t)row[2 * k + 1] << 32) | row[2 * k]);
+    DenominatorAcc acc(seed);
+#pragma unroll
+    for (int j = 0; j < n_args; ++j) {
+        const int32_t c[4] = {(int32_t)row[8 + 4 * j], (int32_t)row[9 + 4 * j], (int32_t)row[10 + 4 * j], (int32_t)row[11 + 4 * j]};
+        acc.add_centred(a[j], c);
+    }
+    return acc.result();
+}
+__device__ __forceinline__ Ext denominator_folded_n(const uint32_t* __restrict__ fold, uint32_t off, const Ext& w, const Ext& al, uint32_t bus_monty,
+                                                    const Ext* __restrict__ blpow, const uint32_t* a, int n_args) {
+#if !defined(__HIP_DEVICE_COMPILE__)
+    if (!fold) {
+        uint32_t row[8 + 4 * 64];
+        if (n_args > 64) return bb::ext_zero();
+        fold_row(w, al, bus_monty, (uint32_t)n_args, blpow, row);
+        return denominator_of_row(row, a, n_args);
+    }
+#endif
+    return denominator_of_row(fold + off, a, n_args);
+}
+template <int NA>
+__device__ __forceinline__ Ext denominator_folded(const uint32_t* __restrict__ fold, uint32_t off, const Ext& w, const Ext& al, uint32_t bus_monty,
+                                                  const Ext* __restrict__ blpow, const uint32_t (&a)[NA]) {
+    return denominator_folded_n(fold, off, w, al, bus_monty, blpow, a, NA);
+}
+__device__ __forceinline__ Ext denominator_folded0(const uint32_t* __restrict__ fold, uint32_t off, const Ext& w, const Ext& al, uint32_t bus_monty) {
+    return denominator_folded_n(fold, off, w, al, bus_monty, nullptr, nullptr, 0);
+}
+__device__ __forceinline__ Ext sub_scaled(const Ext& x, const Ext& w, uint32_t m) {
+    return {{bb::sub(x.c[0], bb::mul(w.c[0], m)), bb::sub(x.c[1], bb::mul(w.c[1], m)), bb::sub(x.c[2], bb::mul(w.c[2], m)), bb::sub(x.c[3], bb::mul(w.c[3], m))}};
 }
 
 __device__ __forceinline__ Ext scale2(const Ext& a, uint32_t x, const Ext& b, uint32_t y) {
diff --git a/powdr_amd/csrc/logup_kernels.hip b/powdr_amd/csrc/logup_kernels.hip
--- a/powdr_amd/csrc/logup_kernels.hip
+++ b/powdr_amd/csrc/logup_kernels.hip
@@ -117,6 +117,21 @@
     }
 }
 
+__global__ __launch_bounds__(kBlock) void quotient_fold_kernel(const LogupInteraction* __restrict__ inter, const uint32_t* __restrict__ gstarts,
+                                                                uint32_t n_groups, uint32_t row_words, const Ext* __restrict__ apow_groups, Ext al,
+                                                                const Ext* __restrict__ blpow, uint32_t* __restrict__ out) {
+    const uint32_t items = (row_words - 8u) / 4u + 1u;
+    const uint32_t t = blockIdx.x * kBlock + threadIdx.x, g = t / items, item = t % items;
+    if (g >= n_groups) return;
+    const uint32_t i0 = gstarts[g], n = gstarts[g + 1] - i0;
+    if (n < 1 || n > 2) return;
+    const LogupInteraction it = inter[i0];
+    if (item > it.n_args) return;
+    uint32_t* row = out + (size_t)g * row_words;
+    if (item == 0) pwj::fold_seeds(apow_groups[g], al, it.bus_monty, row);
+    else pwj::fold_coefficient(apow_groups[g], blpow[item], row + 8 + 4 * (item - 1));
+}
+
 template <bool XBC, bool FAST, bool PUB>
 __global__ __launch_bounds__(kBlock) void quotient_logup_kernel(const uint32_t* __restrict__ lde, const uint32_t* __restrict__ plde,
                                                                  size_t N, const uint32_t* __restrict__ bytecode,
@@ -364,4 +379,23 @@
     return (int)hipGetLastError();
 }
 
-}
+int quotient_fold_table(const LogupInteraction* d_inter, const uint32_t* d_gstarts, uint32_t n_groups, uint32_t row_words, const bb::Ext* d_apow_groups,
+                        bb::Ext al, const bb::Ext* d_blpow, uint32_t* d_out) {
+    if (!n_groups) return 0;
+    const size_t lanes = (size_t)n_groups * ((row_words - 8u) / 4u + 1u);
+    ScopedKernelTimer t("quotient_fold_kernel");
+    hipLaunchKernelGGL(quotient_fold_kernel, dim3(div_up(lanes, kBlock)), dim3(kBlock), 0, stream(), d_inter, d_gstarts, n_groups, row_words, d_apow_groups, al,
+                       d_blpow, d_out);
+    return (int)hipGetLastError();
+}
+
+void quotient_fold_table_host(const LogupInteraction* inter, const uint32_t* gstarts, uint32_t n_groups, uint32_t row_words, const bb::Ext* apow_groups,
+                              bb::Ext al, const bb::Ext* blpow, uint32_t* out) {
+    for (uint32_t g = 0; g < n_groups; ++g) {
+        const uint32_t i0 = gstarts[g], n = gstarts[g + 1] - i0;
+        if (n < 1 || n > 2) continue;
+        pwj::fold_row(apow_groups[g], al, inter[i0].bus_monty, inter[i0].n_args, blpow, out + (size_t)g * row_words);
+    }
+}
+
+}
diff --git a/powdr_amd/csrc/prover.hip b/powdr_amd/csrc/prover.hip
--- a/powdr_amd/csrc/prover.hip
+++ b/powdr_amd/csrc/prover.hip
@@ -1,6 +1,7 @@
 #include "prover_state.hpp"
 #include "prover_stages.hpp"
 #include "xbc_compile.hpp"
+#include "jit_device.hpp"
 
 #include <atomic>
 #include <cstdlib>
@@ -356,6 +357,29 @@
     return u.source.size();
 }
 
+extern "C" size_t pw_quotient_fold_table_host(const uint32_t* inter, size_t n_inter, const uint32_t* ispans, size_t n_ispans, const uint32_t* ibc,
+                                              size_t ibc_len, const uint32_t* apow_groups, const uint32_t* alpha_l, const uint32_t* blpow,
+                                              uint32_t* out, size_t cap_words, uint32_t* row_words) {
+    uint32_t max_args = 0;
+    if (!inter || !n_inter || !apow_groups || !alpha_l || !blpow || !pw::interaction_table_ok(inter, n_inter, ispans, n_ispans, ibc_len, &max_args)) return 0;
+    for (size_t i = 0; i < n_inter; ++i)
+        for (uint32_t k = 0; k <= inter[3 * i + 1]; ++k) {
+            const uint32_t* sp = ispans + 2 * ((size_t)inter[3 * i + 2] + k);
+            if (pw::postfix_degree(ibc + sp[0], sp[1]) == pw::kBadDegree) return 0;
+        }
+    const std::vector<uint32_t> gstarts = pw::logup_group_starts(inter, n_inter, ispans, ibc);
+    const uint32_t n_groups = (uint32_t)gstarts.size() - 1, words = pwj::fold_row_words(max_args);
+    if (row_words) *row_words = words;
+    if (!out || cap_words < (size_t)n_groups * words) return 0;
+    std::vector<pw::LogupInteraction> li(n_inter);
+    for (size_t i = 0; i < n_inter; ++i) li[i] = {bb::to_monty(inter[3 * i] % bb::P), inter[3 * i + 1], 0};
+    bb::Ext al;
+    memcpy(&al, alpha_l, sizeof al);
+    pw::quotient_fold_table_host(li.data(), gstarts.data(), n_groups, words, reinterpret_cast<const bb::Ext*>(apow_groups), al,
+                                 reinterpret_cast<const bb::Ext*>(blpow), out);
+    return n_groups;
+}
+
 #define TRY(x) do { int _rc = (x); if (_rc) return _rc; } while (0)
 
 extern "C" int pw_prover_logup_path(const PwProver* p) { return !p || !p->logup ? 0 : p->d_iforms ? 2 : 1; }
@@ -568,7 +592,7 @@
 
 extern "C" void pw_prover_destroy(PwProver* p) {
     if (!p) return;
-    for (DeviceBuf* b : {&p->coef, &p->lde, &p->digests, &p->q, &p->qcoef, &p->qlde, &p->ext_arena, &p->misc, &p->perm, &p->plde, &p->qpart, &p->tcoef,
+    for (DeviceBuf* b : {&p->coef, &p->lde, &p->digests, &p->q, &p->qcoef, &p->qlde, &p->ext_arena, &p->misc, &p->perm, &p->plde, &p->qpart, &p->qfold, &p->tcoef,
                          &p->fscale, &p->gbuf, &p->pre_vals, &p->pre_lde, &p->pre_tree, &p->row_vals, &p->bus_order})
         b->release();
     if (p->d_next_cols) (void)hipFree(p->d_next_cols);
@@ -600,7 +624,7 @@
 
 extern "C" size_t pw_prover_device_bytes(const PwProver* p) {
     return p->coef.bytes + p->lde.bytes + p->digests.bytes + p->q.bytes + p->qcoef.bytes + p->qlde.bytes +
-           p->ext_arena.bytes + p->misc.bytes + p->perm.bytes + p->plde.bytes + p->qpart.bytes + p->tcoef.bytes + p->fscale.bytes + p->gbuf.bytes +
+           p->ext_arena.bytes + p->misc.bytes + p->perm.bytes + p->plde.bytes + p->qpart.bytes + p->qfold.bytes + p->tcoef.bytes + p->fscale.bytes + p->gbuf.bytes +
            p->pre_vals.bytes + p->pre_lde.bytes + p->pre_tree.bytes + p->row_vals.bytes + p->bus_order.bytes;
 }
 
diff --git a/powdr_amd/csrc/prover_internal.hpp b/powdr_amd/csrc/prover_internal.hpp
--- a/powdr_amd/csrc/prover_internal.hpp
+++ b/powdr_amd/csrc/prover_internal.hpp
@@ -117,6 +117,10 @@
 int quotient_eval_logup(const uint32_t* lde, const uint32_t* plde, size_t N, int logN, const ConstraintProgram& prog,
                         const LogupProgram& lp, const bb::Ext* d_apow, bb::Ext al, const bb::Ext* d_blpow, bb::Ext S,
                         uint32_t zval_even, uint32_t zval_odd, uint32_t* q, bool main_only = false);
+int quotient_fold_table(const LogupInteraction* d_inter, const uint32_t* d_gstarts, uint32_t n_groups, uint32_t row_words, const bb::Ext* d_apow_groups,
+                        bb::Ext al, const bb::Ext* d_blpow, uint32_t* d_out);
+void quotient_fold_table_host(const LogupInteraction* inter, const uint32_t* gstarts, uint32_t n_groups, uint32_t row_words, const bb::Ext* apow_groups,
+                              bb::Ext al, const bb::Ext* blpow, uint32_t* out);
 int deep_quotient_logup(const uint32_t* lde, uint32_t W, const uint32_t* plde, uint32_t Wp, const uint32_t* qlde, size_t N, int logN,
                         const bb::Ext* d_gpow, bb::Ext sum1, bb::Ext sum2, bb::Ext zeta, bb::Ext gzeta, bb::Ext* v);
 int deep_quotient_two_point(const uint32_t* lde, uint32_t W, const uint32_t* plde, uint32_t Wp, const uint32_t* qlde, size_t N, int logN,
diff --git a/powdr_amd/csrc/prover_jit.hip b/powdr_amd/csrc/prover_jit.hip
--- a/powdr_amd/csrc/prover_jit.hip
+++ b/powdr_amd/csrc/prover_jit.hip
@@ -131,12 +131,38 @@
     return a > b ? a : b;
 }
 
+size_t jit_fold_bytes(const PwProver* p) {
+    return p->jit.state == 1 && p->jit.quotient.has_fold ? (size_t)(p->n_groups ? p->n_groups : 1) * p->jit.quotient.fold_row_words * 4 : 0;
+}
+
+int quotient_fold_jit(PwProver* p, const bb::Ext* d_apow, bb::Ext al, const bb::Ext* d_blpow) {
+    const size_t bytes = jit_fold_bytes(p);
+    if (!bytes) return 0;
+    PW_TRY_INT(p->qfold.ensure(bytes));
+    return quotient_fold_table(p->d_inter, p->d_gstarts, p->n_groups, p->jit.quotient.fold_row_words, d_apow + p->n_constraints, al, d_blpow,
+                               p->qfold.as<uint32_t>());
+}
+
+namespace {
+struct QuotientTail {
+    const uint32_t* pub;
+    const uint32_t* fold;
+    void* slot[2];
+    QuotientTail(PwProver* p, const jit::Generated& g) : pub(p->d_pub), fold(p->qfold.as<uint32_t>()) {
+        int k = 0;
+        slot[0] = slot[1] = (void*)&pub;
+        if (g.has_pub) slot[k++] = (void*)&pub;
+        if (g.has_fold) slot[k++] = (void*)&fold;
+    }
+};
+}
+
 int quotient_parts_jit(PwProver* p, const uint32_t* T, const uint32_t* Pm, size_t rows, const bb::Ext* d_apow, bb::Ext al, const bb::Ext* d_blpow,
                        uint32_t* part, uint32_t* n_chunks) {
     const jit::Generated& g = p->jit.quotient;
     uint64_t n64 = rows;
-    const uint32_t* pub = p->d_pub;
-    void* args[] = {(void*)&T, (void*)&Pm, (void*)&n64, (void*)&d_apow, (void*)&al, (void*)&d_blpow, (void*)&part, (void*)&pub};
+    QuotientTail tail(p, g);
+    void* args[] = {(void*)&T, (void*)&Pm, (void*)&n64, (void*)&d_apow, (void*)&al, (void*)&d_blpow, (void*)&part, tail.slot[0], tail.slot[1]};
     ScopedKernelTimer t(Pm ? "quotient_logup_jit_kernel" : "quotient_jit_kernel");
     const int rc = launch_units(g, p->jit.quotient_prog, rows, args);
     if (n_chunks) *n_chunks = g.n_chunks;
@@ -157,8 +183,8 @@
                       const bb::Ext* d_blpow, uint32_t* part) {
     const jit::Generated& g = p->jit.quotient;
     uint64_t n64 = rows;
-    const uint32_t* pub = p->d_pub;
-    void* args[] = {(void*)&T, (void*)&Pm, (void*)&n64, (void*)&d_apow, (void*)&al, (void*)&d_blpow, (void*)&part, (void*)&pub};
+    QuotientTail tail(p, g);
+    void* args[] = {(void*)&T, (void*)&Pm, (void*)&n64, (void*)&d_apow, (void*)&al, (void*)&d_blpow, (void*)&part, tail.slot[0], tail.slot[1]};
     ScopedKernelTimer t(Pm ? "quotient_logup_jit_kernel" : "quotient_jit_kernel");
     return launch_unit(g, p->jit.quotient_prog, u, rows, args);
 }
diff --git a/powdr_amd/csrc/prover_stages.hpp b/powdr_amd/csrc/prover_stages.hpp
--- a/powdr_amd/csrc/prover_stages.hpp
+++ b/powdr_amd/csrc/prover_stages.hpp
@@ -57,9 +57,9 @@
 }
 
 struct BufferPlan {
-    size_t coef = 0, lde = 0, digests = 0, tcoef = 0, fscale = 0, perm = 0, plde = 0, q = 0, qpart = 0, qcoef = 0, qlde = 0, gbuf = 0,
+    size_t coef = 0, lde = 0, digests = 0, tcoef = 0, fscale = 0, perm = 0, plde = 0, q = 0, qpart = 0, qfold = 0, qcoef = 0, qlde = 0, gbuf = 0,
            ext_arena = 0, misc = 0;
-    size_t total() const { return coef + lde + digests + tcoef + fscale + perm + plde + q + qpart + qcoef + qlde + gbuf + ext_arena + misc; }
+    size_t total() const { return coef + lde + digests + tcoef + fscale + perm + plde + q + qpart + qfold + qcoef + qlde + gbuf + ext_arena + misc; }
     BufferPlan commit_part() const { BufferPlan C; C.coef = coef; C.lde = lde; C.digests = digests; C.tcoef = tcoef; C.fscale = fscale; return C; }
 };
 
@@ -87,6 +87,7 @@
     }
     if (b) B.qpart += 4 * L.m * 4;
     B.qpart = std::max(B.qpart, jit_part_bytes(p, H, q_rows));
+    if (lg) B.qfold = jit_fold_bytes(p);
     if (b && m.eat && lg) {
         B.perm = std::max(B.perm, (size_t)s.W * H * 4);
         B.lde = std::max(B.lde, (size_t)(s.Wp + kJitExtraPermCols) * H * 4);
@@ -98,7 +99,7 @@
 inline int apply_plan(PwProver* p, const BufferPlan& B) {
     const struct { DeviceBuf* buf; size_t bytes; } all[] = {
         {&p->coef, B.coef}, {&p->lde, B.lde}, {&p->digests, B.digests}, {&p->tcoef, B.tcoef}, {&p->fscale, B.fscale}, {&p->perm, B.perm},
-        {&p->plde, B.plde}, {&p->q, B.q}, {&p->qpart, B.qpart}, {&p->qcoef, B.qcoef}, {&p->qlde, B.qlde}, {&p->ext_arena, B.ext_arena},
+        {&p->plde, B.plde}, {&p->q, B.q}, {&p->qpart, B.qpart}, {&p->qfold, B.qfold}, {&p->qcoef, B.qcoef}, {&p->qlde, B.qlde}, {&p->ext_arena, B.ext_arena},
         {&p->misc, B.misc}, {&p->gbuf, B.gbuf}};
     for (const auto& e : all)
         if (e.bytes) PW_STRY(e.buf->ensure(e.bytes));
@@ -154,6 +155,7 @@
     uint32_t* d_lde = p->lde.as<uint32_t>();
     uint32_t* d_plde = p->plde.as<uint32_t>();
     uint32_t* d_q = p->q.as<uint32_t>();
+    if (lg && jit) PW_STRY(quotient_fold_jit(p, B.apow, al, B.blpow));
     if (m.b) {
         PW_STRY(streamed::quotient_sums(stream_ctx(p, s, L), jit, lg, s.nc, prog, logup_program(p, s), B.tcoef, p->perm.as<uint32_t>(), B.apow, al,
                                         B.blpow, S, s.logN, d_q));
diff --git a/powdr_amd/csrc/prover_state.hpp b/powdr_amd/csrc/prover_state.hpp
--- a/powdr_amd/csrc/prover_state.hpp
+++ b/powdr_amd/csrc/prover_state.hpp
@@ -91,6 +91,7 @@
     int committed_b = 0;
     pw::DeviceBuf coef, lde, digests, q, qcoef, qlde, ext_arena, misc;
     pw::DeviceBuf qpart;
+    pw::DeviceBuf qfold;
     pw::DeviceBuf tcoef, fscale, gbuf;
     struct OpenedMailbox {
         static constexpr int kEvents = 8;
@@ -156,6 +157,8 @@
                       const bb::Ext* d_blpow, uint32_t* part);
 uint32_t quotient_max_unit_perm_cols(const PwProver* p);
 size_t jit_part_bytes(const PwProver* p, size_t H, size_t q_rows);
+size_t jit_fold_bytes(const PwProver* p);
+int quotient_fold_jit(PwProver* p, const bb::Ext* d_apow, bb::Ext al, const bb::Ext* d_blpow);
 int quotient_eval_logup_jit(PwProver* p, const uint32_t* lde, const uint32_t* plde, size_t N, int logN, const bb::Ext* d_apow, bb::Ext al,
                             const bb::Ext* d_blpow, bb::Ext S, uint32_t zval_even, uint32_t zval_odd, uint32_t* q);
 int logup_perm_trace_jit(PwProver* p, const uint32_t* trace, size_t H, bb::Ext al, const bb::Ext* d_blpow, uint32_t* perm, bb::Ext* d_rowsum,
diff --git a/powdr_amd/prover.py b/powdr_amd/prover.py
--- a/powdr_amd/prover.py
+++ b/powdr_amd/prover.py
@@ -15,7 +15,7 @@
 
 PROVER_SYMBOLS = ["pw_prover_check_constraints", "pw_verify", "pw_prover_create", "pw_prover_create_logup", "pw_verify_logup", "pw_prover_trace_root", "pw_prover_set_bus_seed", "pw_prover_logup_path", "pw_prove_airs", "pw_verify_airs", "pw_prove_segment", "pw_verify_segment", "pw_commitment_digest", "pw_logup_group_starts", "pw_prover_width", "pw_prover_reserve", "pw_prover_stream_log_blocks", "pw_prover_max_constraint_degree", "pw_prover_destroy", "pw_prover_prove", "pw_prover_prove_consuming", "pw_prover_stream_log_blocks_consuming", "pw_trace_from_coefficients", "pw_prover_device_bytes",
                   "pw_lde_batch", "pw_lde_fused", "pw_lde_subcoset", "pw_merkle_commit", "pw_poseidon2_permute_host",
-                  "pw_set_poseidon2_constants", "pw_get_poseidon2_constants", "pw_prover_specialise", "pw_prover_specialised", "pw_jit_compile_check", "pw_jit_cache_stats", "pw_jit_generated_source",
+                  "pw_set_poseidon2_constants", "pw_get_poseidon2_constants", "pw_prover_specialise", "pw_prover_specialised", "pw_jit_compile_check", "pw_jit_cache_stats", "pw_jit_generated_source", "pw_quotient_fold_table_host",
                   "pw_prove_segments_multi", "pw_multi_last_merge", "pw_assign_units",
                   "pw_prove_segment_consuming", "pw_segment_last_modes", "pw_segment_last_plan", "pw_set_device_budget", "pw_get_device_budget", "pw_provers_specialise",
                   "pw_segment_context_bytes", "pw_segment_stream_plan", "pw_segment_last_plan_tables",
@@ -573,6 +573,26 @@
     return units, total.value
 
 
+def quotient_fold_table_host(interactions, apow_groups, alpha_l, blpow) -> np.ndarray:
+    f = lib.pw_quotient_fold_table_host
+    f.restype = C.c_size_t
+    f.argtypes = [C.c_void_p, C.c_size_t, C.c_void_p, C.c_size_t, C.c_void_p, C.c_size_t, C.c_void_p, C.c_void_p, C.c_void_p, C.c_void_p, C.c_size_t,
+                  C.POINTER(C.c_uint32)]
+    tables, _ = _interaction_tables(interactions)
+    a, l, b = (np.ascontiguousarray(x, dtype=np.uint32) for x in (apow_groups, alpha_l, blpow))
+    words = C.c_uint32()
+    f(*tables, _vp(a), _vp(l), _vp(b), None, 0, C.byref(words))
+    if words.value == 0:
+        raise ValueError("malformed interaction table")
+    n_groups = len(logup_group_starts(interactions)) - 1
+    if a.size != 4 * n_groups or l.size != 4 or b.size < words.value - 4:
+        raise ValueError("apow_groups: one extension element per group; blpow: beta^0 .. beta^(most arguments)")
+    out = np.zeros((n_groups, words.value), np.uint32)
+    if f(*tables, _vp(a), _vp(l), _vp(b), _vp(out), out.size, C.byref(words)) != n_groups:
+        raise ValueError("malformed interaction table")
+    return out
+
+
 def jit_cache_stats() -> dict:
     lib.pw_jit_cache_stats.restype = None
     lib.pw_jit_cache_stats.argtypes = [C.POINTER(C.c_uint64), C.POINTER(C.c_uint64)]
diff --git a/rust/powdr-hip/src/ffi.rs b/rust/powdr-hip/src/ffi.rs
--- a/rust/powdr-hip/src/ffi.rs
+++ b/rust/powdr-hip/src/ffi.rs
@@ -442,6 +442,9 @@
                                    inter_bytecode: *const u32, inter_bytecode_len: usize, which: c_int, chunk_cost: u32, chunks_per_unit: u32,
                                    unit: usize, buf: *mut c_char, cap: usize, kernel_name: *mut c_char, name_cap: usize, first_chunk: *mut u32,
                                    n_chunks: *mut u32, total_chunks: *mut u32) -> usize;
+    pub fn pw_quotient_fold_table_host(interactions: *const u32, n_interactions: usize, inter_spans: *const u32, n_inter_spans: usize,
+                                       inter_bytecode: *const u32, inter_bytecode_len: usize, apow_groups: *const u32, alpha_l: *const u32,
+                                       blpow: *const u32, out: *mut u32, cap_words: usize, row_words: *mut u32) -> usize;
     pub fn pw_jit_cache_stats(units_compiled: *mut u64, units_from_disk: *mut u64);
     pub fn pw_jit_compile_check(width: u32, cons_bytecode: *const u32, bytecode_len: usize, cons_spans: *const u32, n_constraints: usize,
                                 interactions: *const u32, n_interactions: usize, inter_spans: *const u32, n_inter_spans: usize,
```

Result: no change. 7.190 billion, median of 6 (+0.8%).
